# phuang1024/Starst3r

Hardware: AMD Instinct MI355X
Metric: 3DGS train iters/sec @ 1M Gaussians, 8x1080p views (higher is better)
Workload: dtype f32

## Files before the change

starst3r_amd/csrc/api.hip:

```cpp
#include <stdarg.h>

#include "common.h"

static thread_local char g_err[512] = "";

void st3r_set_error(const char* fmt, ...) {
    va_list ap;
    va_start(ap, fmt);
    vsnprintf(g_err, sizeof(g_err), fmt, ap);
    va_end(ap);
}

ST3R_EXPORT int st3r_version(void) { return ST3R_VERSION; }
ST3R_EXPORT const char* st3r_last_error(void) { return g_err; }

ST3R_EXPORT int st3r_ctx_create(int device, st3r_ctx** out) {
    ARG_CHECK(out);
    int ndev = 0;
    HIP_TRY(hipGetDeviceCount(&ndev));
    ARG_CHECK(device >= 0 && device < ndev);
    HIP_TRY(hipSetDevice(device));
    st3r_ctx* c = new (std::nothrow) st3r_ctx();
    if (!c) { st3r_set_error("out of host memory"); return ST3R_ERR_NOMEM; }
    memset(c, 0, sizeof(*c));
    c->device = device;
    hipError_t e = hipHostMalloc((void**)&c->pinned, 64 * sizeof(int64_t), hipHostMallocDefault);
    if (e != hipSuccess) { delete c; st3r_set_error("hipHostMalloc: %s", hipGetErrorString(e)); return ST3R_ERR_HIP; }
    *out = c;
    return ST3R_OK;
}

ST3R_EXPORT int st3r_ctx_destroy(st3r_ctx* ctx) {
    if (!ctx) return ST3R_OK;
    (void)hipSetDevice(ctx->device);
    (void)st3r_comm_destroy(ctx);
    for (int i = 0; i < SLOT_COUNT; ++i)
        if (ctx->slot_ptr[i]) (void)hipFree(ctx->slot_ptr[i]);
    if (ctx->pinned) (void)hipHostFree(ctx->pinned);
    if (ctx->count_event) (void)hipEventDestroy(ctx->count_event);
    if (ctx->peer_event) (void)hipEventDestroy(ctx->peer_event);
    if (ctx->comm_stream) {
        for (int j = 0; j < ST3R_MAX_RANGES; ++j) {
            (void)hipEventDestroy(ctx->ev_range_bwd[j]); (void)hipEventDestroy(ctx->ev_range_red[j]);
        }
        (void)hipStreamDestroy(ctx->comm_stream);
    }
    if (ctx->prof_ev[0][0][0])
        for (int r = 0; r < PROF_RING; ++r)
            for (int st = 0; st < STG_COUNT; ++st)
                for (int k = 0; k < 2; ++k) (void)hipEventDestroy(ctx->prof_ev[r][st][k]);
    delete ctx;
    return ST3R_OK;
}

ST3R_EXPORT int64_t st3r_ctx_arena_bytes(st3r_ctx* ctx) {
    if (!ctx) return 0;
    int64_t t = 0;
    for (int i = 0; i < SLOT_COUNT; ++i) t += (int64_t)ctx->slot_bytes[i];
    return t;
}

int st3r_arena_get(st3r_ctx* ctx, int slot, size_t bytes, void** out) {
    int grown;
    return st3r_arena_get2(ctx, slot, bytes, out, &grown);
}

int st3r_arena_get2(st3r_ctx* ctx, int slot, size_t bytes, void** out, int* grown) {
    *grown = 0;
    if (bytes == 0) bytes = 16;
    if (ctx->slot_bytes[slot] < bytes) {
        size_t want = bytes + bytes / 4;
        want = (want + 255) & ~(size_t)255;
        if (ctx->slot_ptr[slot]) {
            HIP_TRY(hipDeviceSynchronize());
            HIP_TRY(hipFree(ctx->slot_ptr[slot]));
            ctx->slot_ptr[slot] = nullptr; ctx->slot_bytes[slot] = 0;
        }
        hipError_t e = hipMalloc(&ctx->slot_ptr[slot], want);
        if (e != hipSuccess) {
            st3r_set_error("arena slot %d: hipMalloc(%zu) failed: %s", slot, want, hipGetErrorString(e));
            return ST3R_ERR_NOMEM;
        }
        ctx->slot_bytes[slot] = want;
        *grown = 1;
    }
    *out = ctx->slot_ptr[slot];
    return ST3R_OK;
}

ST3R_EXPORT int st3r_ctx_peek(st3r_ctx* ctx, void* stream, int which, void* dst, int64_t bytes) {
    ARG_CHECK(ctx && dst && bytes >= 0 && which >= 0 && which <= 10);
    static const int slots[11] = {SLOT_VALS_B, SLOT_OFFSETS, SLOT_SPLATS, SLOT_CUM,
                                  SLOT_MCMC_CUM, SLOT_MCMC_DEAD, SLOT_MCMC_SAMPLED, SLOT_MCMC_COUNT,
                                  SLOT_RGB, SLOT_ALPHA, SLOT_COUNTS};
    ARG_CHECK((size_t)bytes <= ctx->slot_bytes[slots[which]]);
    HIP_TRY(hipMemcpyAsync(dst, ctx->slot_ptr[slots[which]], (size_t)bytes, hipMemcpyDeviceToDevice,
                           (hipStream_t)stream));
    return ST3R_OK;
}

static const char* k_stage_names[STG_COUNT] = {"project", "scan", "emit", "sort", "offsets", "blend_fwd", "loss",
                                               "blend_bwd", "project_bwd", "adam", "sort_depth"};

ST3R_EXPORT const char* st3r_stage_name(int stage) {
    return (stage >= 0 && stage < STG_COUNT) ? k_stage_names[stage] : "";
}

static void prof_harvest_slot(st3r_ctx* ctx, int slot) {
    for (int st = 0; st < STG_COUNT; ++st) {
        if (!ctx->prof_used[slot][st]) continue;
        float ms = 0.f;
        if (hipEventSynchronize(ctx->prof_ev[slot][st][1]) == hipSuccess &&
            hipEventElapsedTime(&ms, ctx->prof_ev[slot][st][0], ctx->prof_ev[slot][st][1]) == hipSuccess) {
            ctx->prof_ms[st] += ms; ctx->prof_n[st] += 1;
        }
        ctx->prof_used[slot][st] = 0;
    }
}

void st3r_prof_begin(st3r_ctx* ctx, hipStream_t s, int stage) {
    if (!((ctx->prof_enabled >> stage) & 1)) return;
    (void)hipEventRecord(ctx->prof_ev[ctx->prof_slot][stage][0], s);
}

void st3r_prof_end(st3r_ctx* ctx, hipStream_t s, int stage) {
    if (!((ctx->prof_enabled >> stage) & 1)) return;
    (void)hipEventRecord(ctx->prof_ev[ctx->prof_slot][stage][1], s);
    ctx->prof_used[ctx->prof_slot][stage] = 1;
}

void st3r_prof_next_step(st3r_ctx* ctx) {
    if (!ctx->prof_enabled) return;
    ctx->prof_slot = (ctx->prof_slot + 1) % PROF_RING;
    prof_harvest_slot(ctx, ctx->prof_slot);
}

ST3R_EXPORT int st3r_ctx_set_debug(st3r_ctx* ctx, int flags) {
    ARG_CHECK(ctx);
    ctx->debug_flags = flags;
    return ST3R_OK;
}

ST3R_EXPORT int st3r_ctx_set_profiling(st3r_ctx* ctx, int enable) {
    ARG_CHECK(ctx && enable >= 0 && enable < 2 + STG_COUNT);
    if (enable && !ctx->prof_ev[0][0][0]) {
        for (int r = 0; r < PROF_RING; ++r)
            for (int st = 0; st < STG_COUNT; ++st)
                for (int k = 0; k < 2; ++k) HIP_TRY(hipEventCreate(&ctx->prof_ev[r][st][k]));
    }
    ctx->prof_enabled = enable == 0 ? 0 : (enable == 1 ? (1 << STG_COUNT) - 1 : (1 << (enable - 2)));
    return ST3R_OK;
}

ST3R_EXPORT int st3r_ctx_get_stage_ms(st3r_ctx* ctx, double* ms_out, int64_t* counts_out) {
    ARG_CHECK(ctx && ms_out && counts_out);
    HIP_TRY(hipDeviceSynchronize());
    if (ctx->prof_ev[0][0][0])
        for (int r = 0; r < PROF_RING; ++r) prof_harvest_slot(ctx, r);
    for (int st = 0; st < STG_COUNT; ++st) {
        ms_out[st] = ctx->prof_ms[st]; counts_out[st] = ctx->prof_n[st];
        ctx->prof_ms[st] = 0; ctx->prof_n[st] = 0;
    }
    return ST3R_OK;
}

int st3r_isect_scan_impl(st3r_ctx* ctx, hipStream_t s, int64_t n_pairs, const int32_t* tiles, int32_t* cum,
                         int64_t* n_isects_host, const void* pack_rects, int rect32, uint64_t* pack_out,
                         int32_t** total_dev_out, int32_t* total_copy, int32_t* total_host);
int st3r_isect_emit_impl(hipStream_t s, int N, int C, const float* splats, const int32_t* cum, int tile_size,
                         int tile_w, int tile_h, int64_t* isect_ids, int32_t* flatten_ids);
int st3r_sort_impl(st3r_ctx* ctx, hipStream_t s, int64_t n, int end_bit, int64_t* keys_in, int32_t* vals_in,
                   int64_t* keys_out, int32_t* vals_out);
int st3r_isect_offsets_impl(hipStream_t s, int64_t n_isects, const int64_t* ids, int C, int tile_w, int tile_h,
                            int32_t* offsets);
int st3r_project_impl(st3r_ctx* ctx, hipStream_t s, int N, int C, const float* means, const float* quats, const float* scales,
                      const float* opacities, const float* sh, int sh_stride, const float* viewmats, const float* Ks,
                      const float* campos, int width, int height, int tile_size, float eps2d, float near_plane,
                      float far_plane, float radius_clip, float* splats, int32_t* tiles_per_gauss, double* reg_sums,
                      uint64_t* depth_keys, int32_t* depth_vals, int tight, uint32_t key_base, void* rects, int rect32,
                      int reg_overwrite, double* zero_ptr, int zero_n, uint32_t* krange);
int st3r_sort_depth_seg_impl(st3r_ctx* ctx, hipStream_t s, int64_t N, int C, uint32_t* keys_in, int32_t* vals_in,
                             uint32_t* keys_out, int32_t* vals_out, const uint32_t* krange);
int st3r_isect_emit_chain_impl(st3r_ctx* ctx, hipStream_t s, int N, int C, const int32_t* perm, const void* rects,
                               int rect32, int tile_w, int tile_h, uint32_t* tile_keys, int32_t* vals, int64_t cap);
int st3r_records_prepare_impl(hipStream_t s, int N, int C, const float* splats, int tile_size, int tile_w, int tile_h,
                              int tight, int32_t* tiles, uint64_t* depth_keys, int32_t* depth_vals, uint32_t key_base,
                              void* rects, int rect32);
int st3r_isect_offsets32_impl(hipStream_t s, int64_t n_isects, const uint32_t* keys, int C, int tile_w, int tile_h,
                              int32_t* offsets, const int32_t* n_dev);
int st3r_sort_depth_impl(st3r_ctx* ctx, hipStream_t s, int64_t n, int end_bit, uint64_t* keys_in, int32_t* vals_in,
                         uint64_t* keys_out, int32_t* vals_out);
int st3r_sort_depth32_impl(st3r_ctx* ctx, hipStream_t s, int64_t n, int end_bit, uint32_t* keys_in, int32_t* vals_in,
                           uint32_t* keys_out, int32_t* vals_out);
int st3r_sort_tile_impl(st3r_ctx* ctx, hipStream_t s, int64_t n, int end_bit, uint32_t* keys_in, int32_t* vals_in,
                        uint32_t* keys_out, int32_t* vals_out, const int32_t* n_dev);
int st3r_blend_fwd_impl(st3r_ctx* ctx, hipStream_t s, int C, int W, int H, int tile_w, int tile_h,
                        const float* splats, const int32_t* offsets, const int32_t* flat, int64_t n_isects,
                        float* rgb, float* alpha, int32_t* last_ids, bool for_backward, bool end_in_offsets);
int st3r_blend_bwd_impl(st3r_ctx* ctx, hipStream_t s, int C, int W, int H, int tile_w, int tile_h,
                        const float* splats, const int32_t* offsets, const int32_t* flat, int64_t n_isects,
                        const float* alpha, const int32_t* last_ids, const float* v_rgb, const float* v_alpha,
                        const int32_t* cum, const uint64_t* rects, const uint64_t* rectbase, int tight, int64_t n_pairs,
                        float* v_splats,
                        bool end_in_offsets, st3r_vtile_ref* defer);
int st3r_project_sh_bwd_impl(hipStream_t s, int N, int C, const float* means, const float* quats, const float* scales,
                             const float* opacities, const float* sh, int sh_stride, const float* viewmats,
                             const float* Ks, const float* campos, int width, int height, float eps2d,
                             const float* splats, const float* v_splats, float reg_views, float opac_fac,
                             float scale_fac, float* grads, bool accumulate, int g_begin, int g_end, bool range_major,
                             const st3r_vtile_ref* slots);
int st3r_loss_impl(st3r_ctx* ctx, hipStream_t s, int C, int H, int W, const float* render, const float* gt,
                   float w_l1, float w_ssim, double* sums, float* v_render, bool sums_cleared);

static int bit_length_u32(uint32_t v) { int n = 0; while (v) { ++n; v >>= 1; } return n; }

static int settle_pending_count(st3r_ctx* ctx) {
    if (!ctx->count_pending) return ST3R_OK;
    HIP_TRY(hipEventSynchronize(ctx->count_event));
    ctx->count_pending = 0;
    const int64_t n = (int64_t)((int32_t*)(ctx->pinned + 8))[0];
    if (n < 0) {
        ctx->isect_hint = 0;
        ctx->view_chunks = (ctx->view_chunks > 0 ? ctx->view_chunks : 1) * 2;
        st3r_set_error("the previous step produced more than 2^31 tile intersections: its gradients were incomplete -- "
                       "repeat it (st3r_gs_train_fwd_bwd / st3r_gs_train_step now walk the views in %d chunks)",
                       ctx->view_chunks);
        return ST3R_ERR_CAPACITY;
    }
    if (n > ctx->count_cap) {
        ctx->isect_hint = 0;
        st3r_set_error("the previous step produced %lld tile intersections, more than the %lld its buffers were sized "
                       "for from the step before (+25 %%): its gradients were incomplete and st3r_adam_step / "
                       "st3r_gs_train_step did NOT apply them (the update is guarded on the device) -- repeat that step",
                       (long long)n, (long long)ctx->count_cap);
        return ST3R_ERR_CAPACITY;
    }
    ctx->isect_hint = n;
    return ST3R_OK;
}

int st3r_peer_status_settle(st3r_ctx* ctx);

ST3R_EXPORT int st3r_ctx_settle(st3r_ctx* ctx) {
    ARG_CHECK(ctx);
    int rc = st3r_peer_status_settle(ctx);
    if (rc) return rc;
    return settle_pending_count(ctx);
}

ST3R_EXPORT int st3r_ctx_release_scratch(st3r_ctx* ctx) {
    ARG_CHECK(ctx);
    HIP_TRY(hipDeviceSynchronize());
    const int rc = st3r_ctx_settle(ctx);
    for (int i = 0; i < SLOT_COUNT; ++i) {
        if (ctx->slot_ptr[i]) (void)hipFree(ctx->slot_ptr[i]);
        ctx->slot_ptr[i] = nullptr; ctx->slot_bytes[i] = 0;
    }
    return rc;
}

int st3r_counts_buffer(st3r_ctx* ctx, hipStream_t s, int32_t** out) {
    void* p; int grown = 0;
    int rc = st3r_arena_get2(ctx, SLOT_COUNTS, sizeof(int32_t) * 16, &p, &grown);
    if (rc) return rc;
    if (grown) HIP_TRY(hipMemsetAsync(p, 0, ctx->slot_bytes[SLOT_COUNTS], s));
    *out = (int32_t*)p;
    return ST3R_OK;
}

#define GET(slot, type, count, var)                                                          \
    type* var;                                                                               \
    {                                                                                        \
        void* _p;                                                                            \
        int _rc = st3r_arena_get(ctx, slot, sizeof(type) * (size_t)(count), &_p);            \
        if (_rc) return _rc;                                                                 \
        var = (type*)_p;                                                                     \
    }

struct RasterOut {
    float* splats; int32_t* offsets; int32_t* flat; int32_t* cum; const uint64_t* rects; uint64_t* rectbase;
    int64_t n_isects, n_records, n_isects_ref, n_visible; int tile_w, tile_h;
};

static int rasterize_front(st3r_ctx* ctx, hipStream_t s, int N, int C, const float* means, const float* quats,
                           const float* scales, const float* opacities, const float* sh, int sh_stride,
                           const float* viewmats, const float* Ks, const float* campos, int W, int H,
                           double* reg_sums, int tight, const float* records_in, bool allow_async, RasterOut* o,
                           double* loss_sums = nullptr) {
    const int tile = 16;
    const int tile_w = (W + tile - 1) / tile, tile_h = (H + tile - 1) / tile;
    const int64_t n_pairs = (int64_t)N * C;
    float* splats = const_cast<float*>(records_in);
    if (!records_in) {
        GET(SLOT_SPLATS, float, n_pairs * ST3R_SPLAT_STRIDE, own);
        splats = own;
    }
    GET(SLOT_CUM, int32_t, n_pairs, cum);
    GET(SLOT_OFFSETS, int32_t, (int64_t)C * tile_w * tile_h + 1, offsets);
    const float near_plane = 0.01f, far_plane = 1e10f;
    uint32_t near_bits, far_bits;
    memcpy(&near_bits, &near_plane, 4); memcpy(&far_bits, &far_plane, 4);
    const bool key32 = (C <= 8) && (far_bits - near_bits < 0x1FFFFFFFu);
    const int64_t n_sort = n_pairs;
    GET(SLOT_DKEYS_A, uint64_t, n_sort, dkeys_a);
    GET(SLOT_DKEYS_B, uint64_t, n_sort, dkeys_b);
    GET(SLOT_DVALS_A, int32_t, n_sort, dvals_a);
    GET(SLOT_DVALS_B, int32_t, n_sort, perm);
    const int rect32 = (tile_w <= 255 && tile_h <= 255 && !(ctx->debug_flags & 64)) ? 1 : 0;
    GET(SLOT_RECTS, uint64_t, rect32 ? (n_pairs + 1) / 2 : n_pairs, rects);
    int32_t* counts = nullptr;
    { int rc_ = st3r_counts_buffer(ctx, s, &counts); if (rc_) return rc_; }
    uint32_t* const krange = (key32 && reg_sums && !records_in && !(ctx->debug_flags & 4)) ? (uint32_t*)(counts + 8) : nullptr;
    st3r_prof_begin(ctx, s, STG_PROJECT);
    const uint32_t key_base = key32 ? near_bits : 0u;
    int rc = records_in
                 ? st3r_records_prepare_impl(s, N, C, splats, tile, tile_w, tile_h, tight, nullptr, dkeys_a, dvals_a,
                                             key_base, rects, rect32)
                 : st3r_project_impl(ctx, s, N, C, means, quats, scales, opacities, sh, sh_stride, viewmats, Ks, campos,
                                     W, H, tile, 0.3f, near_plane, far_plane, 0.0f, splats, nullptr, reg_sums, dkeys_a,
                                     dvals_a, tight, key_base, rects, rect32, 1, loss_sums, 2 * C, krange);
    if (!rc && records_in && loss_sums) HIP_TRY(hipMemsetAsync(loss_sums, 0, sizeof(double) * 2 * (size_t)C, s));
    st3r_prof_end(ctx, s, STG_PROJECT);
    if (rc) return rc;
    st3r_prof_begin(ctx, s, STG_SORT_DEPTH);
    const int cam_bits = bit_length_u32((uint32_t)(C - 1));
    rc = krange ? st3r_sort_depth_seg_impl(ctx, s, N, C, (uint32_t*)dkeys_a, dvals_a, (uint32_t*)dkeys_b, perm, krange)
         : key32 ? st3r_sort_depth32_impl(ctx, s, n_sort, 29 + cam_bits, (uint32_t*)dkeys_a, dvals_a, (uint32_t*)dkeys_b,
                                          perm)
                 : st3r_sort_depth_impl(ctx, s, n_sort, 32 + cam_bits, dkeys_a, dvals_a, dkeys_b, perm);
    st3r_prof_end(ctx, s, STG_SORT_DEPTH);
    if (rc) return rc;
    int64_t n_isects = 0;
    st3r_prof_begin(ctx, s, STG_SCAN);
    uint64_t* rectbase = nullptr;
    if (tile_w <= 1023 && tile_h <= 1023 && !(ctx->debug_flags & 64)) {
        GET(SLOT_RECTBASE, uint64_t, n_pairs, rb);
        rectbase = rb;
    }
    const int32_t* n_dev = nullptr;
    const int64_t sig = ((int64_t)N << 34) ^ ((int64_t)C << 26) ^ ((int64_t)W << 13) ^ (int64_t)H;
    const bool async = allow_async && ctx->isect_hint > 0 && ctx->hint_sig == sig;
    int32_t* total_dev = nullptr;
    rc = st3r_isect_scan_impl(ctx, s, n_pairs, nullptr, cum, nullptr, rects, rect32, rectbase, &total_dev,
                              async ? counts : nullptr, async ? (int32_t*)(ctx->pinned + 8) : nullptr);
    st3r_prof_end(ctx, s, STG_SCAN);
    if (rc) return rc;
    if (async) {
        if (!ctx->count_event) HIP_TRY(hipEventCreateWithFlags(&ctx->count_event, hipEventDisableTiming));
        HIP_TRY(hipEventRecord(ctx->count_event, s));
        n_isects = ctx->isect_hint + ctx->isect_hint / 4 + 1024;
        if (ctx->debug_flags & 8) n_isects = ctx->isect_hint / 2;
        if (n_isects > 2147483647LL) n_isects = 2147483647LL;
        ctx->count_pending = 1; ctx->count_cap = n_isects;
        o->n_visible = -1; o->n_isects_ref = -1;
    } else {
        HIP_TRY(hipMemcpyAsync(ctx->pinned, total_dev, sizeof(int32_t), hipMemcpyDeviceToHost, s));
        if (reg_sums) HIP_TRY(hipMemcpyAsync(ctx->pinned + 1, reg_sums + 2, 2 * sizeof(double), hipMemcpyDeviceToHost, s));
        HIP_TRY(hipStreamSynchronize(s));
        n_isects = (int64_t)((int32_t*)ctx->pinned)[0];
        if (n_isects < 0) {
            st3r_set_error("more than 2^31 tile intersections in one call: split the views over more calls / GPUs");
            return ST3R_SPLIT_VIEWS;
        }
        o->n_visible = reg_sums ? (int64_t)((double*)ctx->pinned)[1] : -1;
        o->n_isects_ref = reg_sums ? (int64_t)((double*)ctx->pinned)[2] : n_isects;
        if (allow_async) { ctx->isect_hint = n_isects; ctx->hint_sig = sig; }
    }
    GET(SLOT_KEYS_A, uint32_t, n_isects, tkeys_a);
    GET(SLOT_KEYS_B, uint32_t, n_isects, tkeys_b);
    GET(SLOT_VALS_A, int32_t, n_isects, vals_a);
    GET(SLOT_VALS_B, int32_t, n_isects, vals_b);
    n_dev = total_dev;
    o->n_records = async ? -1 : n_isects;
    if (n_isects > 0) {
        st3r_prof_begin(ctx, s, STG_EMIT);
        rc = st3r_isect_emit_chain_impl(ctx, s, N, C, perm, rects, rect32, tile_w, tile_h, tkeys_a, vals_a, n_isects);
        st3r_prof_end(ctx, s, STG_EMIT);
        if (rc) return rc;
        const int end_bit = bit_length_u32((uint32_t)((int64_t)C * tile_w * tile_h - 1));
        st3r_prof_begin(ctx, s, STG_SORT);
        rc = st3r_sort_tile_impl(ctx, s, n_isects, end_bit, tkeys_a, vals_a, tkeys_b, vals_b, n_dev);
        st3r_prof_end(ctx, s, STG_SORT);
        if (rc) return rc;
    }
    st3r_prof_begin(ctx, s, STG_OFFSETS);
    rc = st3r_isect_offsets32_impl(s, n_isects, tkeys_b, C, tile_w, tile_h, offsets, n_dev);
    st3r_prof_end(ctx, s, STG_OFFSETS);
    if (rc) return rc;
    o->splats = splats; o->offsets = offsets; o->flat = vals_b; o->cum = cum; o->rects = rect32 ? nullptr : rects;
    o->rectbase = rectbase;
    o->n_isects = n_isects;
    o->tile_w = tile_w; o->tile_h = tile_h;
    return ST3R_OK;
}

__global__ void k_finalize_loss(int C, const double* __restrict__ sums, const double* __restrict__ reg_sums,
                                double inv_px, double inv_cnt, double w_l1, double w_ssim, double reg_views,
                                double opac_k, double scale_k, float* __restrict__ loss_out) {
    if (threadIdx.x == 0 && blockIdx.x == 0) {
        double loss = 0;
        for (int c = 0; c < C; ++c) loss += w_l1 * sums[2 * c] * inv_px + w_ssim * (1.0 - sums[2 * c + 1] * inv_cnt);
        loss += reg_views * (opac_k * reg_sums[0] + scale_k * reg_sums[1]);
        loss_out[0] = (float)loss;
    }
}

static int train_views(st3r_ctx* ctx, hipStream_t s, int N, int C, const float* means, const float* quats,
                       const float* scales, const float* opacities, const float* sh, int sh_stride,
                       const float* viewmats, const float* Ks, const float* campos, const float* gt_images, int W, int H,
                       float ssim_fac, float opac_fac, float scale_fac, double* sums, double* reg_sums, bool allow_async,
                       bool accumulate, float* grads, RasterOut* ro_out) {
    const int64_t n_pairs = (int64_t)N * C, n_px = (int64_t)C * H * W;
    RasterOut ro;
    int rc = rasterize_front(ctx, s, N, C, means, quats, scales, opacities, sh, sh_stride, viewmats, Ks, campos, W, H,
                             reg_sums, 1, nullptr, allow_async, &ro, sums);
    if (rc) return rc;
    const bool eio = true;
    GET(SLOT_RGB, float, n_px * 3, rgb);
    GET(SLOT_ALPHA, float, n_px, alpha);
    GET(SLOT_LAST, int32_t, n_px, last);
    GET(SLOT_VRENDER, float, n_px * 3, v_rgb);
    float* const v_splats = nullptr;
    st3r_vtile_ref slots_{}; st3r_vtile_ref* const slots = &slots_;
    st3r_prof_begin(ctx, s, STG_BLEND_FWD);
    rc = st3r_blend_fwd_impl(ctx, s, C, W, H, ro.tile_w, ro.tile_h, ro.splats, ro.offsets, ro.flat, ro.n_isects, rgb,
                             alpha, last, true, eio);
    st3r_prof_end(ctx, s, STG_BLEND_FWD);
    if (rc) return rc;
    st3r_prof_begin(ctx, s, STG_LOSS);
    rc = st3r_loss_impl(ctx, s, C, H, W, rgb, gt_images, 1.0f - ssim_fac, ssim_fac, sums, v_rgb, true);
    st3r_prof_end(ctx, s, STG_LOSS);
    if (rc) return rc;
    st3r_prof_begin(ctx, s, STG_BLEND_BWD);
    rc = st3r_blend_bwd_impl(ctx, s, C, W, H, ro.tile_w, ro.tile_h, ro.splats, ro.offsets, ro.flat, ro.n_isects, alpha,
                             last, v_rgb, nullptr, ro.cum, (ctx->debug_flags & 2) ? nullptr : ro.rects,
                             (ctx->debug_flags & 2) ? nullptr : ro.rectbase, 1, n_pairs, v_splats,
                             eio, slots);
    st3r_prof_end(ctx, s, STG_BLEND_BWD);
    if (rc) return rc;
    st3r_prof_begin(ctx, s, STG_PROJECT_BWD);
    ctx->ranges_recorded = 0;
    if (ctx->n_ranges > 1 && ctx->comm_stream) {
        GET(SLOT_GSTAGE, float, (int64_t)23 * N, gstage);
        const int K = ctx->n_ranges;
        for (int j = 0; j < K && !rc; ++j) {
            const int g0 = (int)((int64_t)N * j / K), g1 = (int)((int64_t)N * (j + 1) / K);
            rc = st3r_project_sh_bwd_impl(s, N, C, means, quats, scales, opacities, sh, sh_stride, viewmats, Ks, campos, W,
                                          H, 0.3f, ro.splats, v_splats, (float)C, opac_fac, scale_fac, gstage, accumulate, g0,
                                          g1, true, slots);
            if (!rc) HIP_TRY(hipEventRecord(ctx->ev_range_bwd[j], s));
        }
        if (!rc) ctx->ranges_recorded = K;
    } else {
        rc = st3r_project_sh_bwd_impl(s, N, C, means, quats, scales, opacities, sh, sh_stride, viewmats, Ks, campos, W, H,
                                      0.3f, ro.splats, v_splats, (float)C, opac_fac, scale_fac, grads, accumulate, 0, -1,
                                      false, slots);
    }
    st3r_prof_end(ctx, s, STG_PROJECT_BWD);
    *ro_out = ro;
    return rc;
}

ST3R_EXPORT int st3r_gs_train_fwd_bwd(st3r_ctx* ctx, void* stream, int N, int C, const float* means,
                                      const float* quats, const float* scales, const float* opacities,
                                      const float* sh, int sh_stride, const float* viewmats, const float* Ks,
                                      const float* campos, const float* gt_images, int width, int height,
                                      float ssim_fac, float opac_fac, float scale_fac, float* grads,
                                      float* loss_out, int64_t* stats_host) {
    ARG_CHECK(ctx && N > 0 && C > 0 && C <= ST3R_MAX_VIEWS && width > 0 && height > 0 && sh_stride >= 12);
    ARG_CHECK((int64_t)N * C < 2147483647LL);
    ARG_CHECK(means && quats && scales && opacities && sh && viewmats && Ks && campos && gt_images && grads && loss_out);
    hipStream_t s = (hipStream_t)stream;
    const int W = width, H = height;
    GET(SLOT_SMALL, double, 2 * (size_t)C + 12, small);
    double* sums = small;
    double* reg_sums = small + 2 * C;
    double* reg_scratch = reg_sums + 4;
    st3r_prof_next_step(ctx);
    int rc = settle_pending_count(ctx);
    if (rc) return rc;
    int chunks = ctx->view_chunks > 0 ? ctx->view_chunks : 1;
    if ((ctx->debug_flags & 32) && chunks < 2) chunks = 2;
    if (chunks > C) chunks = C;
    int64_t st_vis = 0, st_is = 0, st_ref = 0;
    for (;;) {
        st_vis = st_is = st_ref = 0;
        bool first = true;
        for (int k = 0; k < chunks && !rc; ++k) {
            const int c0 = (int)((int64_t)k * C / chunks), c1 = (int)((int64_t)(k + 1) * C / chunks);
            if (c1 == c0) continue;
            double* rs = first ? reg_sums : reg_scratch;
            RasterOut ro;
            rc = train_views(ctx, s, N, c1 - c0, means, quats, scales, opacities, sh, sh_stride, viewmats + 16 * c0,
                             Ks + 9 * c0, campos + 3 * c0, gt_images + (int64_t)c0 * H * W * 3, W, H, ssim_fac, opac_fac,
                             scale_fac, sums + 2 * c0, rs, stats_host == nullptr && chunks == 1 && !ctx->comm, !first, grads,
                             &ro);
            if (!rc) { st_vis += ro.n_visible; st_is += ro.n_records; st_ref += ro.n_isects_ref; }
            first = false;
        }
        if (rc == ST3R_SPLIT_VIEWS && chunks < C) {
            chunks = chunks * 2 < C ? chunks * 2 : C;
            rc = ST3R_OK;
            continue;
        }
        break;
    }
    if (rc == ST3R_SPLIT_VIEWS) rc = ST3R_ERR_INVALID;
    if (rc) return rc;
    if (chunks > 1) ctx->view_chunks = chunks;
    const int Hi = H - 10, Wi = W - 10;
    const double cnt = (Hi > 0 && Wi > 0) ? (double)Hi * Wi * 3 : 0.0;
    hipLaunchKernelGGL(k_finalize_loss, dim3(1), dim3(64), 0, s, C, sums, reg_sums, 1.0 / ((double)H * W * 3),
                       cnt > 0 ? 1.0 / cnt : 0.0, (double)(1.0f - ssim_fac), (double)ssim_fac, (double)C,
                       (double)opac_fac / N, (double)scale_fac / (3.0 * N), loss_out);
    LAUNCH_CHECK();
    if (stats_host) {
        stats_host[0] = st_vis; stats_host[1] = st_is; stats_host[2] = st3r_ctx_arena_bytes(ctx);
        stats_host[3] = st_ref;
    }
    return ST3R_OK;
}

ST3R_EXPORT int st3r_gs_raster_train(st3r_ctx* ctx, void* stream, int N, int C, const float* records,
                                     const float* gt_images, int width, int height, float ssim_fac,
                                     float* v_records, float* loss_out, int64_t* stats_host) {
    ARG_CHECK(ctx && N > 0 && C > 0 && width > 0 && height > 0 && records && gt_images && v_records && loss_out);
    ARG_CHECK(C <= ST3R_MAX_VIEWS && (int64_t)N * C < 2147483647LL);
    hipStream_t s = (hipStream_t)stream;
    const int W = width, H = height;
    const int64_t n_pairs = (int64_t)N * C, n_px = (int64_t)C * H * W;
    GET(SLOT_SMALL, double, 2 * (size_t)C + 8, small);
    double* sums = small;
    double* reg_sums = small + 2 * C;
    HIP_TRY(hipMemsetAsync(reg_sums, 0, sizeof(double) * 4, s));
    st3r_prof_next_step(ctx);
    RasterOut ro;
    int rc = settle_pending_count(ctx);
    if (rc) return rc;
    rc = rasterize_front(ctx, s, N, C, nullptr, nullptr, nullptr, nullptr, nullptr, 0, nullptr, nullptr, nullptr, W, H,
                         nullptr, 1, records, stats_host == nullptr, &ro);
    if (rc == ST3R_SPLIT_VIEWS) rc = ST3R_ERR_INVALID;
    if (rc) return rc;
    GET(SLOT_RGB, float, n_px * 3, rgb);
    GET(SLOT_ALPHA, float, n_px, alpha);
    GET(SLOT_LAST, int32_t, n_px, last);
    GET(SLOT_VRENDER, float, n_px * 3, v_rgb);
    st3r_prof_begin(ctx, s, STG_BLEND_FWD);
    rc = st3r_blend_fwd_impl(ctx, s, C, W, H, ro.tile_w, ro.tile_h, ro.splats, ro.offsets, ro.flat, ro.n_isects, rgb,
                             alpha, last, true, true);
    st3r_prof_end(ctx, s, STG_BLEND_FWD);
    if (rc) return rc;
    st3r_prof_begin(ctx, s, STG_LOSS);
    rc = st3r_loss_impl(ctx, s, C, H, W, rgb, gt_images, 1.0f - ssim_fac, ssim_fac, sums, v_rgb, false);
    st3r_prof_end(ctx, s, STG_LOSS);
    if (rc) return rc;
    st3r_prof_begin(ctx, s, STG_BLEND_BWD);
    rc = st3r_blend_bwd_impl(ctx, s, C, W, H, ro.tile_w, ro.tile_h, ro.splats, ro.offsets, ro.flat, ro.n_isects, alpha,
                             last, v_rgb, nullptr, ro.cum, ro.rects, ro.rectbase, 1, n_pairs, v_records, true, nullptr);
    st3r_prof_end(ctx, s, STG_BLEND_BWD);
    if (rc) return rc;
    const int Hi = H - 10, Wi = W - 10;
    const double cnt = (Hi > 0 && Wi > 0) ? (double)Hi * Wi * 3 : 0.0;
    hipLaunchKernelGGL(k_finalize_loss, dim3(1), dim3(64), 0, s, C, sums, reg_sums, 1.0 / ((double)H * W * 3),
                       cnt > 0 ? 1.0 / cnt : 0.0, (double)(1.0f - ssim_fac), (double)ssim_fac, 0.0, 0.0, 0.0, loss_out);
    LAUNCH_CHECK();
    if (stats_host) {
        stats_host[0] = -1; stats_host[1] = ro.n_records; stats_host[2] = st3r_ctx_arena_bytes(ctx); stats_host[3] = -1;
    }
    return ST3R_OK;
}

ST3R_EXPORT int st3r_gs_render(st3r_ctx* ctx, void* stream, int N, int C, const float* means, const float* quats,
                               const float* scales, const float* opacities, const float* sh, int sh_stride,
                               const float* viewmats, const float* Ks, const float* campos, int width, int height,
                               float* rgb, float* alpha, int64_t* stats_host) {
    ARG_CHECK(ctx && N > 0 && C > 0 && width > 0 && height > 0 && sh_stride >= 12);
    ARG_CHECK(C <= ST3R_MAX_VIEWS && (int64_t)N * C < 2147483647LL);
    ARG_CHECK(means && quats && scales && opacities && sh && viewmats && Ks && campos && rgb && alpha);
    hipStream_t s = (hipStream_t)stream;
    RasterOut ro;
    int rc = settle_pending_count(ctx);
    if (rc) return rc;
    rc = rasterize_front(ctx, s, N, C, means, quats, scales, opacities, sh, sh_stride, viewmats, Ks, campos, width, height,
                         nullptr, 0, nullptr, false, &ro);
    if (rc == ST3R_SPLIT_VIEWS) rc = ST3R_ERR_INVALID;
    if (rc) return rc;
    GET(SLOT_LAST, int32_t, (int64_t)C * height * width, last);
    rc = st3r_blend_fwd_impl(ctx, s, C, width, height, ro.tile_w, ro.tile_h, ro.splats, ro.offsets, ro.flat,
                             ro.n_isects, rgb, alpha, last, false, true);
    if (rc) return rc;
    if (stats_host) {
        stats_host[0] = -1; stats_host[1] = ro.n_records; stats_host[2] = st3r_ctx_arena_bytes(ctx); stats_host[3] = 0;
    }
    return ST3R_OK;
}
```

starst3r_amd/csrc/common.h:

```cpp
#pragma once
#include <hip/hip_runtime.h>
#include <stdint.h>
#include <stdio.h>
#include <string.h>

#include "../../include/st3r.h"

#define ST3R_EXPORT extern "C" __attribute__((visibility("default")))

void st3r_set_error(const char* fmt, ...);

#define HIP_TRY(expr)                                                                              \
    do {                                                                                           \
        hipError_t _e = (expr);                                                                    \
        if (_e != hipSuccess) {                                                                    \
            st3r_set_error("%s:%d: %s -> %s", __FILE__, __LINE__, #expr, hipGetErrorString(_e));   \
            return ST3R_ERR_HIP;                                                                   \
        }                                                                                          \
    } while (0)

#define ARG_CHECK(cond)                                                                    \
    do {                                                                                   \
        if (!(cond)) {                                                                     \
            st3r_set_error("%s:%d: invalid argument: %s", __FILE__, __LINE__, #cond);      \
            return ST3R_ERR_INVALID;                                                       \
        }                                                                                  \
    } while (0)

#define LAUNCH_CHECK() HIP_TRY(hipGetLastError())

enum ArenaSlot {
    SLOT_SPLATS = 0,
    SLOT_TILES,
    SLOT_CUM,
    SLOT_KEYS_A,
    SLOT_KEYS_B,
    SLOT_VALS_A,
    SLOT_VALS_B,
    SLOT_OFFSETS,
    SLOT_RGB,
    SLOT_ALPHA,
    SLOT_LAST,
    SLOT_VRENDER,
    SLOT_VSPLATS,
    SLOT_SSIM_A,
    SLOT_SORT_TMP,
    SLOT_SCAN_TMP,
    SLOT_SMALL,
    SLOT_CMASK,
    SLOT_TILE_NB,
    SLOT_VTILE,
    SLOT_DKEYS_A,
    SLOT_DKEYS_B,
    SLOT_DVALS_A,
    SLOT_DVALS_B,
    SLOT_CUM_D,
    SLOT_NN_PART,
    SLOT_MCMC_CUM,
    SLOT_MCMC_DEAD,
    SLOT_MCMC_RANK,
    SLOT_MCMC_COUNT,
    SLOT_MCMC_SAMPLED,
    SLOT_MCMC_BINOMS,
    SLOT_REG_PART,
    SLOT_RECTS,
    SLOT_RECTS_D,
    SLOT_RECTBASE,
    SLOT_COUNTS,
    SLOT_PSTAGE,
    SLOT_GSTAGE,
    SLOT_ALIGN_CTL,
    SLOT_PAIR_TOUCH,
    SLOT_KRANGE_PART,
    SLOT_SCAN_CHAIN,
    SLOT_POSE_PART,
    SLOT_VTILE_DEPTH,
    SLOT_DEPTH_PART,
    SLOT_COUNT
};

enum Stage {
    STG_PROJECT = 0,
    STG_SCAN,
    STG_EMIT,
    STG_SORT,
    STG_OFFSETS,
    STG_BLEND_FWD,
    STG_LOSS,
    STG_BLEND_BWD,
    STG_PROJECT_BWD,
    STG_ADAM,
    STG_SORT_DEPTH,
    STG_COUNT
};
#define PROF_RING 64
#define ST3R_MAX_RANGES 8

#define ST3R_SPLIT_VIEWS 1000

struct st3r_vtile_ref { const int32_t* cum; const float* vtile; int stamp; unsigned vt_cap; const uint32_t* touch; };

struct st3r_ctx {
    int device;
    void* slot_ptr[SLOT_COUNT];
    size_t slot_bytes[SLOT_COUNT];
    int64_t* pinned;
    int debug_flags;
    const float* gtm_gt; const float* gtm_mom; int gtm_c, gtm_h, gtm_w;
    int bwd_stamp;
    int depth_stamp;
    uint32_t scan_gen;
    int64_t isect_hint, count_cap;
    int64_t hint_sig;
    int count_pending;
    int view_chunks;
    hipEvent_t count_event;
    void* comm;
    int comm_owned, comm_rank, comm_size;
    int exchange;
    int comm_broken;
    int peer_pending;
    hipEvent_t peer_event;
    hipStream_t comm_stream;
    hipEvent_t ev_range_bwd[ST3R_MAX_RANGES], ev_range_red[ST3R_MAX_RANGES];
    void* xwin;
    int n_ranges;
    int ranges_recorded;
    int prof_enabled;
    hipEvent_t prof_ev[PROF_RING][STG_COUNT][2];
    unsigned char prof_used[PROF_RING][STG_COUNT];
    int prof_slot;
    double prof_ms[STG_COUNT];
    int64_t prof_n[STG_COUNT];
};

void st3r_prof_begin(st3r_ctx* ctx, hipStream_t s, int stage);
void st3r_prof_end(st3r_ctx* ctx, hipStream_t s, int stage);
void st3r_prof_next_step(st3r_ctx* ctx);

int st3r_arena_get(st3r_ctx* ctx, int slot, size_t bytes, void** out);
int st3r_arena_get2(st3r_ctx* ctx, int slot, size_t bytes, void** out, int* grown);

static inline int ceil_div(int64_t a, int64_t b) { return (int)((a + b - 1) / b); }
```

starst3r_amd/csrc/gs_blend.hip:

```cpp
#include <type_traits>

#include "common.h"
#include "tile_rect.h"
#include "blend_common.h"



struct TileGeom {
    int lb, cam, i, j, start, end, tx0, ty0;
    bool inside;
    float px, py;
};

__device__ __forceinline__ TileGeom tile_geom(int C, int W, int H, int tile_w, int tile_h,
                                              const int32_t* __restrict__ offsets, int n_isects) {
    TileGeom g;
    const int n_tiles = tile_w * tile_h, total = C * n_tiles;
        g.lb = xcd_remap(blockIdx.x, total, XCD_GROUP(C, n_tiles, tile_w));
    g.cam = g.lb / n_tiles;
    const int tile = g.lb - g.cam * n_tiles;
    const int ty = tile / tile_w, tx = tile - ty * tile_w;
    g.tx0 = tx * 16; g.ty0 = ty * 16;
    const int w = threadIdx.x >> 6, lane = threadIdx.x & 63;
    g.j = g.tx0 + ((w & 1) << 3) + (lane & 7);
    g.i = g.ty0 + ((w >> 1) << 3) + (lane >> 3);
    g.inside = (g.i < H) && (g.j < W);
    g.px = (float)g.j + 0.5f; g.py = (float)g.i + 0.5f;
    g.start = offsets[g.lb];
    g.end = (g.lb == total - 1 && n_isects >= 0) ? n_isects : offsets[g.lb + 1];
    return g;
}

__device__ __forceinline__ int stage_record(const float4* __restrict__ splats, int64_t id, int t, int tx0, int ty0,
                                            float4* sR) {
    const float4 a = splats[id * 3 + 0];
    const float4 b = splats[id * 3 + 1];
    const float4 c = splats[id * 3 + 2];
    stage_qform(a, b, c, t, sR);
    EllipseTest et;
    if (!ellipse_prepare(a.z, a.w, b.x, b.y, &et)) return 0;
    const float rx = ((float)tx0 + 0.5f) - a.x, ry = ((float)ty0 + 0.5f) - a.y;
    int rel = 0;
#pragma unroll
    for (int q = 0; q < 4; ++q) {
        const float dx0 = rx + (float)((q & 1) * 8), dy0 = ry + (float)((q >> 1) * 8);
        rel |= ellipse_hits_square(et, dx0, dx0 + 7.0f, dy0, dy0 + 7.0f) ? (1 << q) : 0;
    }
    return rel;
}

template <bool TRAIN>
__global__ __launch_bounds__(BLK) void k_blend_fwd(int C, int W, int H, int tile_w, int tile_h,
                                                   const float4* __restrict__ splats,
                                                   const int32_t* __restrict__ offsets,
                                                   const int32_t* __restrict__ flat, int n_isects,
                                                   float* __restrict__ out_rgb, float* __restrict__ out_alpha,
                                                   int32_t* __restrict__ last_ids,
                                                   uint64_t* __restrict__ cmask, int64_t cmask_words,
                                                   int32_t* __restrict__ tile_nb, int no_cull) {
    __shared__ float4 sR[BLK * 3];
    __shared__ uint64_t sMask[4][4];
    const TileGeom g = tile_geom(C, W, H, tile_w, tile_h, offsets, n_isects);
    const int w = threadIdx.x >> 6, lane = threadIdx.x & 63;
    float thr = g.inside ? 1.f / 255.f : __builtin_inff();
    float T = 1.0f, r = 0.f, gg = 0.f, b = 0.f;
    int cur = TRAIN ? 0x7fffffff : 0;
    int nb = 0;
    const int64_t mbase = mask_base(g.lb, g.start);
    for (int bs = g.start; bs < g.end; bs += BLK, ++nb) {
        if (__syncthreads_and(thr > 1.0f)) break;
        const int idx = bs + threadIdx.x;
        int rel = 0;
        if (idx < g.end) {
            rel = stage_record(splats, flat[idx], threadIdx.x, g.tx0, g.ty0, sR);
            if (no_cull) rel = 0xF;
        }
        const uint64_t m0 = __ballot(rel & 1), m1 = __ballot(rel & 2), m2 = __ballot(rel & 4), m3 = __ballot(rel & 8);
        if (lane == 0) { sMask[0][w] = m0; sMask[1][w] = m1; sMask[2][w] = m2; sMask[3][w] = m3; }
        __syncthreads();
#pragma unroll 1
        for (int jj = 0; jj < 4; ++jj) {
            uint64_t m64 = uniform_u64(sMask[w][jj]);
            uint64_t contributed = 0;
            if (__builtin_amdgcn_ballot_w64(thr < 1.0f) == 0) m64 = 0;
#pragma unroll 1
            for (int hh = 0; hh < 2; ++hh) {
            uint32_t m = hh ? (uint32_t)(m64 >> 32) : (uint32_t)m64;
            uint32_t cont32 = 0;
            while (m) {
                const int bit = __builtin_ctz(m);
                m &= m - 1;
                const int t = jj * 64 + hh * 32 + bit;
                const float4 a = sR[3 * t];
                const float4 q = sR[3 * t + 1];
                const float cb = sR[3 * t + 2].x;
                const float dx = a.x - g.px, dy = a.y - g.py;
                const float P = blend_power(dx, dy, a.w, q.x, q.y);
                const float al0 = fminf(0.999f, a.z * __builtin_amdgcn_exp2f(P));
                uint64_t okm = 0;
                bool ok = false;
                float al;
                if (TRAIN) {
                    okm = mask_not_positive(P) & mask_not_less(al0, thr);
                    al = zero_unless(okm, al0);
                } else {
                    ok = !(P > 0.f) && !(al0 < thr);
                    al = ok ? al0 : 0.f;
                }
                const float nT = T * (1.0f - al);
                const bool stop = nT <= 1e-4f;
                float vis = al * T;
                uint64_t tm;
                if (TRAIN) {
                    tm = okm;
                    float Tn = nT;
                    if (__builtin_expect(__builtin_amdgcn_ballot_w64(stop) != 0, 0)) {
                        thr = stop ? __builtin_inff() : thr;
                        vis = stop ? 0.0f : vis;
                        Tn = stop ? T : nT;
                        cur = stop ? bs + t : cur;
                        tm = okm & ~__builtin_amdgcn_ballot_w64(stop);
                    }
                    T = Tn;
                } else {
                    thr = stop ? __builtin_inff() : thr;
                    al = stop ? 0.0f : al;
                    vis = al * T;
                    T = stop ? T : nT;
                    const bool took = al > 0.0f;
                    cur = took ? bs + t : cur;
                    tm = __builtin_amdgcn_ballot_w64(took);
                }
                r = __builtin_fmaf(q.z, vis, r); gg = __builtin_fmaf(q.w, vis, gg); b = __builtin_fmaf(cb, vis, b);
                cont32 |= tm ? (1u << bit) : 0u;
            }
            contributed |= (uint64_t)cont32 << (32 * hh);
            }
            if (cmask && lane == 0) cmask[(int64_t)w * cmask_words + mbase + nb * 4 + jj] = contributed;
        }
    }
    if (g.inside) {
        const int64_t p = ((int64_t)g.cam * H + g.i) * W + g.j;
        out_rgb[3 * p] = r; out_rgb[3 * p + 1] = gg; out_rgb[3 * p + 2] = b;
        out_alpha[p] = 1.0f - T;
        last_ids[p] = TRAIN ? (cur == 0x7fffffff ? cur : cur - 1) : cur;
    }
    if (tile_nb && threadIdx.x == 0) tile_nb[g.lb] = nb;
}

static int hand_off_buffers(st3r_ctx* ctx, int C, int tile_w, int tile_h, int64_t n_isects, uint64_t** cmask,
                            int64_t* words, int32_t** tile_nb) {
    const int64_t total = (int64_t)C * tile_w * tile_h;
    *words = (n_isects >> 6) + 4 * total + 8;
    void* p;
    int rc = st3r_arena_get(ctx, SLOT_CMASK, sizeof(uint64_t) * 4 * (size_t)*words, &p);
    if (rc) return rc;
    *cmask = (uint64_t*)p;
    rc = st3r_arena_get(ctx, SLOT_TILE_NB, sizeof(int32_t) * (size_t)total, &p);
    if (rc) return rc;
    *tile_nb = (int32_t*)p;
    return ST3R_OK;
}

int st3r_blend_fwd_cells_impl(st3r_ctx* ctx, hipStream_t s, int C, int W, int H, int tile_w, int tile_h,
                              const float* splats, const int32_t* offsets, const int32_t* flat, float* rgb, float* alpha,
                              int32_t* last_ids, uint64_t* cmask, int64_t cmask_words, int32_t* tile_nb);

int st3r_blend_fwd_impl(st3r_ctx* ctx, hipStream_t s, int C, int W, int H, int tile_w, int tile_h,
                        const float* splats, const int32_t* offsets, const int32_t* flat, int64_t n_isects,
                        float* rgb, float* alpha, int32_t* last_ids, bool for_backward, bool end_in_offsets) {
    const int total = C * tile_w * tile_h;
    uint64_t* cmask = nullptr; int64_t words = 0; int32_t* tile_nb = nullptr;
    if (for_backward) {
        int rc = hand_off_buffers(ctx, C, tile_w, tile_h, n_isects, &cmask, &words, &tile_nb);
        if (rc) return rc;
    }
    if ((for_backward && end_in_offsets && !(ctx->debug_flags & 128)) || (end_in_offsets && (ctx->debug_flags & 512)))
        return st3r_blend_fwd_cells_impl(ctx, s, C, W, H, tile_w, tile_h, splats, offsets, flat, rgb, alpha, last_ids, cmask,
                                         words, tile_nb);
    if (for_backward && end_in_offsets)
        hipLaunchKernelGGL(k_blend_fwd<true>, dim3(total), dim3(BLK), 0, s, C, W, H, tile_w, tile_h, (const float4*)splats,
                           offsets, flat, -1, rgb, alpha, last_ids, cmask, words, tile_nb, ctx->debug_flags & 1);
    else
        hipLaunchKernelGGL(k_blend_fwd<false>, dim3(total), dim3(BLK), 0, s, C, W, H, tile_w, tile_h, (const float4*)splats,
                           offsets, flat, end_in_offsets ? -1 : (int)n_isects, rgb, alpha, last_ids, cmask, words, tile_nb,
                           ctx->debug_flags & 1);
    LAUNCH_CHECK();
    return ST3R_OK;
}

ST3R_EXPORT int st3r_gs_blend_fwd(st3r_ctx* ctx, void* stream, int C, int width, int height, int tile_size,
                                  int tile_w, int tile_h, const float* splats, const int32_t* offsets,
                                  const int32_t* flatten_ids, int64_t n_isects, float* rgb, float* alpha,
                                  int32_t* last_ids) {
    ARG_CHECK(ctx && C > 0 && width > 0 && height > 0 && tile_size == 16);
    ARG_CHECK(tile_w == (width + 15) / 16 && tile_h == (height + 15) / 16);
    ARG_CHECK(splats && offsets && rgb && alpha && last_ids && n_isects >= 0 && n_isects < 2147483647LL);
    ARG_CHECK(n_isects == 0 || flatten_ids);
    return st3r_blend_fwd_impl(ctx, (hipStream_t)stream, C, width, height, tile_w, tile_h, splats, offsets,
                               flatten_ids, n_isects, rgb, alpha, last_ids, true, false);
}

__device__ __forceinline__ void bwd_phase2(const float2* __restrict__ pr, unsigned tpack, int cnt, int lane, const float4* sA, float* accw, float qxf_lane, float qyf_lane,
                                           const float (&pvr)[CHUNK], const float (&pvg)[CHUNK],
                                           const float (&pvb)[CHUNK]) {
    static_assert(CHUNK == 4, "one DPP row per record of the chunk");
    const int r = lane >> 4, part = lane & 15;
    wave_lds_sync();
    const int t = (tpack >> (8 * r)) & 0xFF;
    const float2 mean = *reinterpret_cast<const float2*>(&sA[t]);
    const float dy = mean.y - qyf_lane;
    const float2* src = pr + r * PAIR_STRIDE + PAIR_AT(part * CHUNK);
    float W0 = 0.f, W1 = 0.f, W2 = 0.f, Sr = 0.f, Sg = 0.f, Sb = 0.f;
#pragma unroll
    for (int i = 0; i < CHUNK; ++i) {
        const float2 v = src[i];
        W0 += v.x;
        if (i == 1) { W1 = v.x; W2 = v.x; }
        if (i > 1) { W1 = fmaf((float)i, v.x, W1); W2 = fmaf((float)(i * i), v.x, W2); }
        Sr = fmaf(v.y, pvr[i], Sr); Sg = fmaf(v.y, pvg[i], Sg); Sb = fmaf(v.y, pvb[i], Sb);
    }
    const float d0 = mean.x - qxf_lane;
    const float So = W0, Sx = fmaf(d0, W0, -W1), Sxx = fmaf(d0, Sx - W1, W2);
    const float Sy = So * dy, Sxy = Sx * dy, Syy = Sy * dy;
    float k0, k1, k2;
    reduce9_rows(Sx, Sy, So, Sxx, Sxy, Syy, Sr, Sg, Sb, k0, k1, k2);
    if (r < cnt && (lane & 3) == 0) {
        const int b = (lane >> 2) & 3;
        const int slot0 = ((b & 1) << 1) | (b >> 1);
        float* acc = accw + t * ACC_VALS;
        acc[slot0] = k0;
        acc[4 + slot0] = k1;
        if (b == 0) acc[8] = k2;
    }
    wave_lds_sync();
}

template <bool HAS_VA, bool TOUCH = false>
__global__ __launch_bounds__(BLK) __attribute__((amdgpu_waves_per_eu(8))) void k_blend_bwd(int C, int W, int H, int tile_w, int tile_h,
                                                   const float4* __restrict__ splats,
                                                   const int32_t* __restrict__ offsets,
                                                   const int32_t* __restrict__ flat, int n_isects,
                                                   const float* __restrict__ out_alpha,
                                                   const int32_t* __restrict__ last_ids,
                                                   const float* __restrict__ v_rgb,
                                                   const float* __restrict__ v_alpha,
                                                   const uint64_t* __restrict__ cmask, int64_t cmask_words,
                                                   const int32_t* __restrict__ tile_nb,
                                                   const int32_t* __restrict__ cum,
                                                   const uint64_t* __restrict__ rects,
                                                   const uint64_t* __restrict__ rectbase, int tight,
                                                   float* __restrict__ vtile, int stamp, unsigned vt_cap) {

    __shared__ float4 sA[HB];
    __shared__ float4 sB[HB];
    __shared__ float sC[HB];
    __shared__ float sAccW[4][HB * ACC_VALS];
    __shared__ float2 sPair[4][CHUNK * PAIR_STRIDE];
    __shared__ uint64_t sClampW;
    const TileGeom g = tile_geom(C, W, H, tile_w, tile_h, offsets, n_isects);
    const int nb = tile_nb[g.lb];
    if (nb == 0) return;
    const int w = threadIdx.x >> 6, lane = threadIdx.x & 63;
    const int64_t p = ((int64_t)g.cam * H + g.i) * W + g.j;
    float T_final = 1.0f, vr = 0.f, vg = 0.f, vb = 0.f, va = 0.f;
    int bin_final = -1;
    if (g.inside) {
        T_final = 1.0f - out_alpha[p];
        vr = v_rgb[3 * p]; vg = v_rgb[3 * p + 1]; vb = v_rgb[3 * p + 2];
        if (HAS_VA) va = v_alpha[p];
        bin_final = last_ids[p];
    }
    const bool chk_index = __builtin_amdgcn_ballot_w64(bin_final != 0x7fffffff) != 0;
    float2* pr = sPair[w];
    float* accw = sAccW[w];
    float pvr[CHUNK], pvg[CHUNK], pvb[CHUNK];
    const int pbase = (lane & 15) * CHUNK;
    {
        float* px = reinterpret_cast<float*>(pr);
        px[lane] = vr; px[64 + lane] = vg; px[128 + lane] = vb;
        wave_lds_sync();
#pragma unroll
        for (int i = 0; i < CHUNK; ++i) { pvr[i] = px[pbase + i]; pvg[i] = px[64 + pbase + i]; pvb[i] = px[128 + pbase + i]; }
        wave_lds_sync();
    }
    const float qxf = (float)(g.tx0 + ((w & 1) << 3) + (pbase & 7)) + 0.5f;
    const float qyf_part = (float)(g.ty0 + ((w >> 1) << 3) + (pbase >> 3)) + 0.5f;
    float k_big = 0x1p64f, k_neg_thr = -__int_as_float(0x3b808080) * 0x1p64f;
    asm volatile("" : "+v"(k_big), "+v"(k_neg_thr));
    float T = T_final;
    float bv = 0.f;
    const int64_t mbase = mask_base(g.lb, g.start);
    const uint64_t* wmask = cmask + (int64_t)__builtin_amdgcn_readfirstlane(w) * cmask_words + mbase;
    uint64_t m_next = wmask[(BLK / HB) * nb - 1];
    for (int hb = (BLK / HB) * nb - 1; hb >= 0; --hb) {
        const int bs = g.start + hb * HB;
        const int bsz = min(HB, g.end - bs);
        const uint64_t m_cur = m_next;
        if (hb > 0) m_next = wmask[hb - 1];
        if (bsz <= 0) continue;
        int my_u = -1, my_cb = 0;
        float my_op = 0.f, my_ca = 0.f, my_cbb = 0.f, my_cc = 0.f;
        if ((int)threadIdx.x < bsz) {
            const int t = threadIdx.x;
            const int64_t my_id = flat[bs + t];
            const int64_t word = mbase + hb;
#pragma unroll
            for (int ww = 0; ww < 4; ++ww) my_cb |= (int)((cmask[ww * cmask_words + word] >> (t & 63)) & 1ull) << ww;
            float4 a = make_float4(0.f, 0.f, 0.f, 0.f), b = a, c = a;
            if (my_cb)
            {
                a = splats[my_id * 3 + 0];
                b = splats[my_id * 3 + 1];
                c = splats[my_id * 3 + 2];
                sA[t] = make_float4(a.x, a.y, a.z, -0.5f * LOG2E * a.w);
                sB[t] = make_float4(-LOG2E * b.x, -0.5f * LOG2E * b.y, b.z, b.w);
                sC[t] = c.x;
            }
            const float det_ = a.w * b.y - b.x * b.x;
            const bool hard = my_cb && !(a.z <= 0.998f && a.w > 0.f && b.y > 0.f && det_ >= 2e-3f * (a.w * b.y));
            const uint64_t cw = __builtin_amdgcn_ballot_w64(hard);
            if (t == 0) sClampW = cw;
            if (my_cb && rectbase) {
                if (TOUCH) reinterpret_cast<uint32_t*>(const_cast<uint64_t*>(rects))[my_id] = (uint32_t)stamp;
                const uint64_t r = rectbase[my_id];
                const int x0 = (int)(r & 0x3FF), y0 = (int)((r >> 10) & 0x3FF), rw = (int)((r >> 20) & 0x3FF);
                my_u = (int)(r >> 32) + ((g.ty0 >> 4) - y0) * rw + ((g.tx0 >> 4) - x0);
                my_op = a.z; my_ca = a.w; my_cbb = b.x; my_cc = b.y;
            } else if (my_cb) {
                int x0, y0, rw;
                if (rects) {
                    const uint64_t r = rects[my_id];
                    x0 = (int)(r & 0xFFFF); y0 = (int)((r >> 16) & 0xFFFF); rw = (int)((r >> 32) & 0xFFFF);
                } else {
                    TileRect tr = ref_tile_rect(a.x, a.y, (float)__float_as_int(c.z), 16, tile_w, tile_h);
                    if (tight) tr = tight_tile_rect(tr, a.x, a.y, a.z, a.w, b.x, b.y);
                    x0 = tr.x0; y0 = tr.y0; rw = tr.x1 - tr.x0;
                }
                const int cum_excl = my_id == 0 ? 0 : cum[my_id - 1];
                my_u = cum_excl + ((g.ty0 >> 4) - y0) * rw + ((g.tx0 >> 4) - x0);
                my_op = a.z; my_ca = a.w; my_cbb = b.x; my_cc = b.y;
            }
        }
        __syncthreads();
        auto walk = [&](auto chk_tag, auto clamp_tag) {
            constexpr bool CHK = decltype(chk_tag)::value, CLAMP = decltype(clamp_tag)::value;
            uint64_t m = m_cur;
            while (m) {
                unsigned tpack = 0;
                int cnt = 0;
#pragma unroll
                for (int k = 0; k < CHUNK; ++k) {
                    if (m) {
                        const int t = 63 - __builtin_clzll(m);
                        m &= ~(1ull << t);
                        const float4 a = sA[t];
                        const float4 q = sB[t];
                        const float cb_ = sC[t];
                        const float dx = a.x - g.px, dy = a.y - g.py;
                        const float P = blend_power(dx, dy, a.w, q.x, q.y);
                        const float vis0 = __builtin_amdgcn_exp2f(P);
                        const float ov0 = a.z * vis0;
                        float alpha;
                        if (CLAMP) {
                            const float al0 = fminf(0.999f, ov0);
                            uint64_t okm = mask_not_positive(P) & mask_not_less(al0, 1.f / 255.f);
                            if (CHK) okm &= __builtin_amdgcn_ballot_w64(bs + t <= bin_final);
                            alpha = zero_unless(okm, al0);
                        } else {
                            float step;
                            asm("v_fma_f32 %0, %1, %2, %3 clamp" : "=v"(step) : "v"(ov0), "v"(k_big), "v"(k_neg_thr));
                            alpha = ov0 * step;
                            if (CHK) alpha = zero_unless(__builtin_amdgcn_ballot_w64(bs + t <= bin_final), alpha);
                        }
                        float alpha_u = alpha;
                        if (CLAMP) alpha_u = ov0 <= 0.999f ? alpha : 0.f;
                        const float ra = __builtin_amdgcn_rcpf(1.0f - alpha);
                        const float cv = q.z * vr + q.w * vg + cb_ * vb;
                        T *= ra;
                        const float fac = alpha * T;
                        float v_al = cv * T - bv * ra;
                        if (HAS_VA) v_al += T_final * ra * va;
                        bv += cv * fac;
                        pr[k * PAIR_STRIDE + PAIR_AT(lane)] = make_float2(alpha_u * v_al, fac);
                        tpack |= (unsigned)t << (8 * k);
                        cnt = k + 1;
                    }
                }
                bwd_phase2(pr, tpack, cnt, lane, sA, accw, qxf, qyf_part, pvr, pvg, pvb);
            }
        };
        const bool clamp_round = (uniform_u64(sClampW) & m_cur) != 0;
        if (chk_index) {
            if (clamp_round) walk(std::true_type{}, std::true_type{}); else walk(std::true_type{}, std::false_type{});
        } else {
            if (clamp_round) walk(std::false_type{}, std::true_type{}); else walk(std::false_type{}, std::false_type{});
        }
        __syncthreads();
        if (my_cb && (unsigned)my_u < vt_cap) {
            float acc[ACC_VALS];
#pragma unroll
            for (int k = 0; k < ACC_VALS; ++k) acc[k] = 0.f;
#pragma unroll
            for (int ww = 0; ww < 4; ++ww) {
                if (my_cb & (1 << ww)) {
#pragma unroll
                    for (int k = 0; k < ACC_VALS; ++k) acc[k] += sAccW[ww][threadIdx.x * ACC_VALS + k];
                }
            }
            const float sx = -acc[0], sy = -acc[1];
            float2* dst = reinterpret_cast<float2*>(vtile + (int64_t)my_u * VT_STRIDE);
            dst[0] = make_float2(my_ca * sx + my_cbb * sy, my_cbb * sx + my_cc * sy);
            dst[1] = make_float2(my_op != 0.f ? acc[2] / my_op : 0.f, -0.5f * acc[3]);
            dst[2] = make_float2(-acc[4], -0.5f * acc[5]);
            dst[3] = make_float2(acc[6], acc[7]);
            dst[4] = make_float2(acc[8], __int_as_float(stamp));
        }
    }
}

__global__ __launch_bounds__(256) void k_gather_vtile(int64_t n_pairs, const int32_t* __restrict__ cum,
                                                      const float* __restrict__ vtile, int stamp, unsigned vt_cap,
                                                      float4* __restrict__ v_splats) {
    constexpr int ROW = ACC_VALS;
    __shared__ int sCum[257];
    __shared__ float sVal[256 * ROW];
    const int tid = threadIdx.x;
    const int64_t p0 = (int64_t)blockIdx.x * 256;
    const int np = (int)min((int64_t)256, n_pairs - p0);
    if (tid == 0) sCum[0] = p0 == 0 ? 0 : cum[p0 - 1];
    sCum[tid + 1] = cum[p0 + min(tid, np - 1)];
    __syncthreads();
    const int s0 = sCum[0], s1 = sCum[np];
    const int my_start = sCum[tid], my_end = tid < np ? sCum[tid + 1] : sCum[tid];
    float acc[ACC_VALS];
#pragma unroll
    for (int k = 0; k < ACC_VALS; ++k) acc[k] = 0.f;
    float2 q0, q1, q2, q3, q4;
    auto fetch = [&](int u) {
        q0 = q1 = q2 = q3 = q4 = make_float2(0.f, 0.f);
        if (u < s1 && (unsigned)u < vt_cap) {
            const float2* src = reinterpret_cast<const float2*>(vtile + (int64_t)u * VT_STRIDE);
            q0 = src[0]; q1 = src[1]; q2 = src[2]; q3 = src[3]; q4 = src[4];
        }
    };
    fetch(s0 + tid);
    for (int base = s0; base < s1; base += 256) {
        const bool live = __float_as_int(q4.y) == stamp;
        float* row = sVal + tid * ROW;
        row[0] = live ? q0.x : 0.f; row[1] = live ? q0.y : 0.f; row[2] = live ? q1.x : 0.f;
        row[3] = live ? q1.y : 0.f; row[4] = live ? q2.x : 0.f; row[5] = live ? q2.y : 0.f;
        row[6] = live ? q3.x : 0.f; row[7] = live ? q3.y : 0.f; row[8] = live ? q4.x : 0.f;
        __syncthreads();
        fetch(base + 256 + tid);
        const int lo = max(my_start, base) - base, hi = min(my_end, base + 256) - base;
        for (int r = lo; r < hi; ++r) {
            const float* src = sVal + r * ROW;
#pragma unroll
            for (int k = 0; k < ACC_VALS; ++k) acc[k] += src[k];
        }
        __syncthreads();
    }
    if (tid < np) {
        const int64_t pid = p0 + tid;
        v_splats[pid * 3 + 0] = make_float4(acc[0], acc[1], acc[2], acc[3]);
        v_splats[pid * 3 + 1] = make_float4(acc[4], acc[5], acc[6], acc[7]);
        v_splats[pid * 3 + 2] = make_float4(acc[8], 0.f, 0.f, 0.f);
    }
}

int st3r_blend_bwd_impl(st3r_ctx* ctx, hipStream_t s, int C, int W, int H, int tile_w, int tile_h,
                        const float* splats, const int32_t* offsets, const int32_t* flat, int64_t n_isects,
                        const float* alpha, const int32_t* last_ids, const float* v_rgb, const float* v_alpha,
                        const int32_t* cum, const uint64_t* rects, const uint64_t* rectbase, int tight, int64_t n_pairs,
                        float* v_splats, bool end_in_offsets, st3r_vtile_ref* defer) {
    if (defer) *defer = st3r_vtile_ref{cum, nullptr, 0, 0u, nullptr};
    if (n_isects == 0) {
        if (!defer) HIP_TRY(hipMemsetAsync(v_splats, 0, sizeof(float) * ST3R_SPLAT_STRIDE * (size_t)n_pairs, s));
        return ST3R_OK;
    }
    uint64_t* cmask; int64_t words; int32_t* tile_nb;
    int rc = hand_off_buffers(ctx, C, tile_w, tile_h, n_isects, &cmask, &words, &tile_nb);
    if (rc) return rc;
    void* p; int grown = 0;
    rc = st3r_arena_get2(ctx, SLOT_VTILE, sizeof(float) * VT_STRIDE * (size_t)n_isects, &p, &grown);
    if (rc) return rc;
    float* vtile = (float*)p;
    uint32_t* touch = nullptr;
    int grown_t = 0;
    if (defer && rectbase && !v_alpha && n_isects > 8 * n_pairs) {
        void* pt;
        rc = st3r_arena_get2(ctx, SLOT_PAIR_TOUCH, sizeof(uint32_t) * (size_t)n_pairs, &pt, &grown_t);
        if (rc) return rc;
        touch = (uint32_t*)pt;
    }
    if (grown || ctx->bwd_stamp >= 2147483000) {
        HIP_TRY(hipMemsetAsync(p, 0, ctx->slot_bytes[SLOT_VTILE], s));
        if (ctx->slot_ptr[SLOT_PAIR_TOUCH])
            HIP_TRY(hipMemsetAsync(ctx->slot_ptr[SLOT_PAIR_TOUCH], 0, ctx->slot_bytes[SLOT_PAIR_TOUCH], s));
        ctx->bwd_stamp = 0;
    } else if (grown_t) {
        HIP_TRY(hipMemsetAsync(touch, 0, ctx->slot_bytes[SLOT_PAIR_TOUCH], s));
    }
    const int stamp = ++ctx->bwd_stamp;
    const int total = C * tile_w * tile_h;
    const unsigned vt_cap = (unsigned)(ctx->slot_bytes[SLOT_VTILE] / (sizeof(float) * VT_STRIDE));
    if (v_alpha)
        hipLaunchKernelGGL(k_blend_bwd<true>, dim3(total), dim3(BLK), 0, s, C, W, H, tile_w, tile_h,
                           (const float4*)splats, offsets, flat, end_in_offsets ? -1 : (int)n_isects, alpha, last_ids, v_rgb,
                           v_alpha, cmask, words, tile_nb, cum, rects, rectbase, tight, vtile, stamp, vt_cap);
    else if (touch)
        hipLaunchKernelGGL((k_blend_bwd<false, true>), dim3(total), dim3(BLK), 0, s, C, W, H, tile_w, tile_h,
                           (const float4*)splats, offsets, flat, end_in_offsets ? -1 : (int)n_isects, alpha, last_ids, v_rgb,
                           v_alpha, cmask, words, tile_nb, cum, reinterpret_cast<const uint64_t*>(touch), rectbase, tight, vtile,
                           stamp, vt_cap);
    else
        hipLaunchKernelGGL(k_blend_bwd<false>, dim3(total), dim3(BLK), 0, s, C, W, H, tile_w, tile_h,
                           (const float4*)splats, offsets, flat, end_in_offsets ? -1 : (int)n_isects, alpha, last_ids, v_rgb,
                           v_alpha, cmask, words, tile_nb, cum, rects, rectbase, tight, vtile, stamp, vt_cap);
    LAUNCH_CHECK();
    if (defer) { *defer = st3r_vtile_ref{cum, vtile, stamp, vt_cap, touch}; return ST3R_OK; }
    hipLaunchKernelGGL(k_gather_vtile, dim3(ceil_div(n_pairs, 256)), dim3(256), 0, s, n_pairs, cum, vtile, stamp, vt_cap,
                       (float4*)v_splats);
    LAUNCH_CHECK();
    return ST3R_OK;
}

ST3R_EXPORT int st3r_gs_blend_bwd(st3r_ctx* ctx, void* stream, int C, int width, int height, int tile_size,
                                  int tile_w, int tile_h, const float* splats, const int32_t* offsets,
                                  const int32_t* flatten_ids, int64_t n_isects, const float* alpha,
                                  const int32_t* last_ids, const float* v_rgb, const float* v_alpha,
                                  const int32_t* cum_tiles, int64_t n_pairs, float* v_splats) {
    ARG_CHECK(ctx && C > 0 && width > 0 && height > 0 && tile_size == 16);
    ARG_CHECK(tile_w == (width + 15) / 16 && tile_h == (height + 15) / 16);
    ARG_CHECK(splats && offsets && alpha && last_ids && v_rgb && v_splats && cum_tiles && n_pairs >= 0);
    ARG_CHECK(n_isects >= 0 && n_isects < 2147483647LL && (n_isects == 0 || flatten_ids));
    return st3r_blend_bwd_impl(ctx, (hipStream_t)stream, C, width, height, tile_w, tile_h, splats, offsets,
                               flatten_ids, n_isects, alpha, last_ids, v_rgb, v_alpha, cum_tiles, nullptr, nullptr, 0, n_pairs,
                               v_splats, false, nullptr);
}
```

starst3r_amd/csrc/gs_isect.hip:

```cpp
#include "common.h"
#include "tile_rect.h"

#define SCAN_THREADS 256
#define SCAN_ITEMS 16
#define SCAN_TILE (SCAN_THREADS * SCAN_ITEMS)

__device__ __forceinline__ int wave_incl_scan(int v) {
    const int lane = threadIdx.x & 63;
#pragma unroll
    for (int off = 1; off < 64; off <<= 1) {
        int t = __shfl_up(v, off);
        if (lane >= off) v += t;
    }
    return v;
}

__device__ __forceinline__ int block_incl_scan(int v, int* total) {
    __shared__ int wsum[4];
    const int lane = threadIdx.x & 63, w = threadIdx.x >> 6;
    int inc = wave_incl_scan(v);
    if (lane == 63) wsum[w] = inc;
    __syncthreads();
    int base = 0;
#pragma unroll
    for (int i = 0; i < 4; ++i) base += (i < w) ? wsum[i] : 0;
    *total = wsum[0] + wsum[1] + wsum[2] + wsum[3];
    __syncthreads();
    return inc + base;
}

typedef unsigned long long u64;
#define SCAN_PAD(i) ((i) + ((i) >> 5))
#define SC_VALUE_MASK 0xFFFFFFFFFFFFull
__device__ __forceinline__ u64 sc_word(u64 flag, uint32_t gen, u64 v) { return (flag << 62) | ((u64)gen << 48) | (v & SC_VALUE_MASK); }

__device__ __forceinline__ u64 chain_lookback256(const u64* st, int k, uint32_t gen, u64* s_part, int* s_near) {
    const int t = threadIdx.x, lane = t & 63, w = t >> 6;
    u64 excl = 0;
    for (int t0 = k - 1;; t0 -= 256) {
        const int tt = t0 - t;
        u64 wd = sc_word(2, gen, 0);
        if (tt >= 0) {
            unsigned spins = 0;
            for (;;) {
                wd = __hip_atomic_load(st + tt, __ATOMIC_RELAXED, __HIP_MEMORY_SCOPE_AGENT);
                if ((wd >> 62) != 0 && (uint32_t)((wd >> 48) & 0x3FFF) == gen) break;
                __builtin_amdgcn_s_sleep(1);
                if (++spins > (1u << 26)) __builtin_trap();
            }
        }
        const u64 incm = __ballot((wd >> 62) == 2);
        const int nearest = incm ? __builtin_ctzll(incm) : 64;
        u64 val = lane <= nearest ? (wd & SC_VALUE_MASK) : 0ull;
#pragma unroll
        for (int off = 32; off > 0; off >>= 1) val += __shfl_down(val, off);
        if (lane == 0) { s_part[w] = val; s_near[w] = nearest; }
        __syncthreads();
        bool done = false;
#pragma unroll
        for (int ww = 0; ww < 4; ++ww)
            if (!done) { excl += s_part[ww]; done = s_near[ww] < 64; }
        __syncthreads();
        if (done) break;
    }
    return excl;
}

template <bool RECTS, bool PACK>
__global__ __launch_bounds__(SCAN_THREADS) void k_scan_chained(const int32_t* in, const void* __restrict__ rects,
                                                               int rect32, int64_t n, int32_t* out,
                                                               uint64_t* __restrict__ pack_out, u64* status,
                                                               uint32_t* ticket, uint32_t gen,
                                                               int32_t* __restrict__ total_out,
                                                               int32_t* __restrict__ total_copy,
                                                               int32_t* __restrict__ total_host) {
    __shared__ int tile[SCAN_PAD(SCAN_TILE) + 1];
    __shared__ uint32_t s_tile;
    if (threadIdx.x == 0) {
        s_tile = atomicAdd(ticket + (gen & 1u), 1u);
        if (s_tile == 0) __hip_atomic_store(ticket + ((gen & 1u) ^ 1u), 0u, __ATOMIC_RELAXED, __HIP_MEMORY_SCOPE_AGENT);
    }
    __syncthreads();
    const uint32_t tl = s_tile;
    const int64_t base0 = (int64_t)tl * SCAN_TILE;
    if (base0 >= n) return;
    uint32_t geo[PACK ? SCAN_ITEMS : 1];
#pragma unroll
    for (int i = 0; i < SCAN_ITEMS; ++i) {
        const int e = i * SCAN_THREADS + threadIdx.x;
        const int64_t idx = base0 + e;
        int v = 0;
        if (RECTS) {
            uint32_t org = 0, rw = 0, rh = 0;
            if (idx < n) rect_load(rects, rect32, idx, &org, &rw, &rh);
            v = (int)(rw * rh);
            if (PACK) geo[i] = (org & 0x3FF) | (((org >> 16) & 0x3FF) << 10) | ((rw & 0x3FF) << 20);
        } else if (idx < n) v = in[idx];
        tile[SCAN_PAD(e)] = v;
    }
    __syncthreads();
    int v[SCAN_ITEMS];
    int s = 0;
#pragma unroll
    for (int i = 0; i < SCAN_ITEMS; ++i) {
        v[i] = tile[SCAN_PAD(threadIdx.x * SCAN_ITEMS + i)];
        s += v[i];
    }
    int total;
    const int inc = block_incl_scan(s, &total);
    const u64 tot = (u64)(uint32_t)total;
    __shared__ u64 s_part[4];
    __shared__ int s_near[4];
    u64 excl = 0;
    if (tl == 0) {
        if (threadIdx.x == 0) __hip_atomic_store(status, sc_word(2, gen, tot), __ATOMIC_RELAXED, __HIP_MEMORY_SCOPE_AGENT);
    } else {
        if (threadIdx.x == 0) __hip_atomic_store(status + tl, sc_word(1, gen, tot), __ATOMIC_RELAXED, __HIP_MEMORY_SCOPE_AGENT);
        excl = chain_lookback256(status, (int)tl, gen, s_part, s_near);
        if (threadIdx.x == 0)
            __hip_atomic_store(status + tl, sc_word(2, gen, excl + tot), __ATOMIC_RELAXED, __HIP_MEMORY_SCOPE_AGENT);
    }
    if (threadIdx.x == 0 && base0 + SCAN_TILE >= n) {
        const u64 all = excl + tot;
        total_out[0] = all > 2147483647ull ? -1 : (int32_t)all;
        if (total_copy) total_copy[0] = total_out[0];
        if (total_host) __hip_atomic_store(total_host, total_out[0], __ATOMIC_RELAXED, __HIP_MEMORY_SCOPE_SYSTEM);
    }
    const int tile_excl = (int)(uint32_t)excl;
    int run = tile_excl + inc - s;
#pragma unroll
    for (int i = 0; i < SCAN_ITEMS; ++i) {
        run += v[i];
        tile[SCAN_PAD(threadIdx.x * SCAN_ITEMS + i)] = run;
    }
    __syncthreads();
#pragma unroll
    for (int i = 0; i < SCAN_ITEMS; ++i) {
        const int e = i * SCAN_THREADS + threadIdx.x;
        const int64_t idx = base0 + e;
        if (idx < n) {
            out[idx] = tile[SCAN_PAD(e)];
            if (PACK) {
                const uint32_t ex = (uint32_t)(e == 0 ? tile_excl : tile[SCAN_PAD(e - 1)]);
                pack_out[idx] = ((uint64_t)ex << 32) | geo[i];
            }
        }
    }
}

struct ChainCtl { uint32_t* tickets; int32_t* total; u64* status; uint32_t gen; };
static int chain_ctl(st3r_ctx* ctx, hipStream_t s, int64_t nwords, ChainCtl* c) {
    void* p; int grown = 0;
    int rc = st3r_arena_get2(ctx, SLOT_SCAN_CHAIN, sizeof(u64) * ((size_t)nwords + 16), &p, &grown);
    if (rc) return rc;
    if (grown || ctx->scan_gen >= 0x3FFF) {
        HIP_TRY(hipMemsetAsync(p, 0, ctx->slot_bytes[SLOT_SCAN_CHAIN], s));
        ctx->scan_gen = 0;
    }
    u64* ctl = (u64*)p;
    c->gen = ++ctx->scan_gen;
    c->tickets = (uint32_t*)ctl;
    c->total = (int32_t*)(ctl + 4) + (c->gen & 3);
    c->status = ctl + 16;
    return ST3R_OK;
}

int st3r_scan_inclusive_i32(st3r_ctx* ctx, hipStream_t s, const int32_t* in, const void* rects, int rect32, int32_t* out,
                            int64_t n, int32_t** total_dev, uint64_t* pack_out = nullptr, int32_t* total_copy = nullptr,
                            int32_t* total_host = nullptr) {
    const int ntiles = ceil_div(n, SCAN_TILE);
    ChainCtl c;
    int rc = chain_ctl(ctx, s, ntiles, &c);
    if (rc) return rc;
#define SCAN_LAUNCH(R, P)                                                                                                \
    hipLaunchKernelGGL((k_scan_chained<R, P>), dim3(ntiles), dim3(SCAN_THREADS), 0, s, in, rects, rect32, n, out, pack_out, \
                       c.status, c.tickets, c.gen, c.total, total_copy, total_host)
    if (rects && pack_out) SCAN_LAUNCH(true, true);
    else if (rects) SCAN_LAUNCH(true, false);
    else SCAN_LAUNCH(false, false);
#undef SCAN_LAUNCH
    LAUNCH_CHECK();
    if (total_dev) *total_dev = c.total;
    return ST3R_OK;
}

int st3r_isect_scan_impl(st3r_ctx* ctx, hipStream_t s, int64_t n_pairs, const int32_t* tiles, int32_t* cum,
                         int64_t* n_isects_host, const void* pack_rects, int rect32, uint64_t* pack_out,
                         int32_t** total_dev_out, int32_t* total_copy, int32_t* total_host) {
    if (n_pairs == 0) { if (n_isects_host) *n_isects_host = 0; return ST3R_OK; }
    int32_t* total_dev = nullptr;
    int rc = st3r_scan_inclusive_i32(ctx, s, tiles, tiles ? nullptr : pack_rects, rect32, cum, n_pairs, &total_dev,
                                     tiles ? nullptr : pack_out, total_copy, total_host);
    if (rc) return rc;
    if (total_dev_out) *total_dev_out = total_dev;
    if (n_isects_host) {
        int32_t* pin = (int32_t*)ctx->pinned;
        HIP_TRY(hipMemcpyAsync(pin, total_dev, sizeof(int32_t), hipMemcpyDeviceToHost, s));
        HIP_TRY(hipStreamSynchronize(s));
        *n_isects_host = (int64_t)pin[0];
    }
    return ST3R_OK;
}

ST3R_EXPORT int st3r_gs_isect_scan(st3r_ctx* ctx, void* stream, int64_t n_pairs, const int32_t* tiles_per_gauss,
                                   int32_t* cum_tiles, int64_t* n_isects_host) {
    ARG_CHECK(ctx && n_pairs >= 0 && tiles_per_gauss && cum_tiles && n_isects_host);
    return st3r_isect_scan_impl(ctx, (hipStream_t)stream, n_pairs, tiles_per_gauss, cum_tiles, n_isects_host, nullptr,
                                0, nullptr, nullptr, nullptr, nullptr);
}

__global__ __launch_bounds__(256) void k_isect_emit(int N, int64_t n_pairs, const float4* __restrict__ splats,
                                                    const int32_t* __restrict__ cum, int tile_size, int tile_w,
                                                    int tile_h, int tile_n_bits, int64_t* __restrict__ isect_ids,
                                                    int32_t* __restrict__ flatten_ids) {
    const int64_t pid = (int64_t)blockIdx.x * blockDim.x + threadIdx.x;
    if (pid >= n_pairs) return;
    const int end = cum[pid];
    const int start = pid == 0 ? 0 : cum[pid - 1];
    if (end == start) return;
    const float4 r0 = splats[pid * 3 + 0];
    const float4 r2 = splats[pid * 3 + 2];
    const float radius = (float)__float_as_int(r2.z);
    const TileRect tr = ref_tile_rect(r0.x, r0.y, radius, tile_size, tile_w, tile_h);
    const int x0 = tr.x0, y0 = tr.y0, x1 = tr.x1, y1 = tr.y1;
    const int64_t cid = pid / N;
    const int64_t cid_enc = cid << (32 + tile_n_bits);
    const int64_t depth_enc = (int64_t)(uint32_t)__float_as_int(r2.y);
    int cur = start;
    for (int ty = y0; ty < y1; ++ty)
        for (int tx = x0; tx < x1; ++tx) {
            const int64_t tile_id = (int64_t)ty * tile_w + tx;
            isect_ids[cur] = cid_enc | (tile_id << 32) | depth_enc;
            flatten_ids[cur] = (int32_t)pid;
            ++cur;
        }
}

static int bit_length_u32(uint32_t v) { int n = 0; while (v) { ++n; v >>= 1; } return n; }

int st3r_isect_emit_impl(hipStream_t s, int N, int C, const float* splats, const int32_t* cum, int tile_size,
                         int tile_w, int tile_h, int64_t* isect_ids, int32_t* flatten_ids) {
    int64_t n_pairs = (int64_t)N * C;
    if (n_pairs == 0) return ST3R_OK;
    int tile_n_bits = bit_length_u32((uint32_t)(tile_w * tile_h));
    hipLaunchKernelGGL(k_isect_emit, dim3(ceil_div(n_pairs, 256)), dim3(256), 0, s, N, n_pairs, (const float4*)splats,
                       cum, tile_size, tile_w, tile_h, tile_n_bits, isect_ids, flatten_ids);
    LAUNCH_CHECK();
    return ST3R_OK;
}

ST3R_EXPORT int st3r_gs_isect_emit(st3r_ctx* ctx, void* stream, int N, int C, const float* splats,
                                   const int32_t* cum_tiles, int tile_size, int tile_w, int tile_h,
                                   int64_t n_isects, int64_t* isect_ids, int32_t* flatten_ids) {
    ARG_CHECK(ctx && N >= 0 && C > 0 && splats && cum_tiles && tile_size > 0 && tile_w > 0 && tile_h > 0);
    if (n_isects == 0) return ST3R_OK;
    ARG_CHECK(isect_ids && flatten_ids);
    return st3r_isect_emit_impl((hipStream_t)stream, N, C, splats, cum_tiles, tile_size, tile_w, tile_h, isect_ids,
                                flatten_ids);
}

__global__ __launch_bounds__(256) void k_isect_offsets(int64_t n_isects, const int64_t* __restrict__ ids, int C,
                                                       int n_tiles, int tile_n_bits,
                                                       int32_t* __restrict__ offsets) {
    const int64_t idx = (int64_t)blockIdx.x * blockDim.x + threadIdx.x;
    if (idx >= n_isects) return;
    const int64_t hi = ids[idx] >> 32;
    const int64_t id_curr = (hi >> tile_n_bits) * n_tiles + (hi & (((int64_t)1 << tile_n_bits) - 1));
    if (idx == 0) {
        for (int64_t i = 0; i <= id_curr; ++i) offsets[i] = 0;
    } else {
        const int64_t hp = ids[idx - 1] >> 32;
        const int64_t id_prev = (hp >> tile_n_bits) * n_tiles + (hp & (((int64_t)1 << tile_n_bits) - 1));
        if (id_prev != id_curr)
            for (int64_t i = id_prev + 1; i <= id_curr; ++i) offsets[i] = (int32_t)idx;
    }
    if (idx == n_isects - 1) {
        const int64_t total = (int64_t)C * n_tiles;
        for (int64_t i = id_curr + 1; i < total; ++i) offsets[i] = (int32_t)n_isects;
    }
}

int st3r_isect_offsets_impl(hipStream_t s, int64_t n_isects, const int64_t* ids, int C, int tile_w, int tile_h,
                            int32_t* offsets) {
    int n_tiles = tile_w * tile_h;
    if (n_isects == 0) {
        HIP_TRY(hipMemsetAsync(offsets, 0, sizeof(int32_t) * (size_t)C * n_tiles, s));
        return ST3R_OK;
    }
    int tile_n_bits = bit_length_u32((uint32_t)n_tiles);
    hipLaunchKernelGGL(k_isect_offsets, dim3(ceil_div(n_isects, 256)), dim3(256), 0, s, n_isects, ids, C, n_tiles,
                       tile_n_bits, offsets);
    LAUNCH_CHECK();
    return ST3R_OK;
}

ST3R_EXPORT int st3r_gs_offsets(st3r_ctx* ctx, void* stream, int64_t n_isects, const int64_t* isect_ids_sorted,
                                int C, int tile_w, int tile_h, int32_t* offsets) {
    ARG_CHECK(ctx && n_isects >= 0 && C > 0 && tile_w > 0 && tile_h > 0 && offsets);
    ARG_CHECK(n_isects == 0 || isect_ids_sorted);
    return st3r_isect_offsets_impl((hipStream_t)stream, n_isects, isect_ids_sorted, C, tile_w, tile_h, offsets);
}

__global__ __launch_bounds__(256) void k_isect_offsets32(int64_t n_isects, const uint32_t* __restrict__ keys,
                                                         int64_t total, int32_t* __restrict__ offsets,
                                                         const int32_t* __restrict__ n_dev) {
    if (n_dev) n_isects = min(n_isects, (int64_t)max(*n_dev, 0));
    const int64_t tid = (int64_t)blockIdx.x * blockDim.x + threadIdx.x;
    if (n_isects == 0) {
        for (int64_t i = tid; i <= total; i += (int64_t)gridDim.x * blockDim.x) offsets[i] = 0;
        return;
    }
    const int64_t i0 = tid * 4;
    if (i0 >= n_isects) return;
    uint32_t k[4];
    if (i0 + 4 <= n_isects) {
        const uint4 v = *reinterpret_cast<const uint4*>(keys + i0);
        k[0] = v.x; k[1] = v.y; k[2] = v.z; k[3] = v.w;
    } else {
#pragma unroll
        for (int j = 0; j < 4; ++j) k[j] = i0 + j < n_isects ? keys[i0 + j] : 0u;
    }
    int64_t prev = i0 == 0 ? -1 : (int64_t)keys[i0 - 1];
#pragma unroll
    for (int j = 0; j < 4; ++j) {
        const int64_t idx = i0 + j;
        if (idx < n_isects) {
            const int64_t cur = k[j];
            for (int64_t i = prev + 1; i <= cur; ++i) offsets[i] = (int32_t)idx;
            prev = cur;
            if (idx == n_isects - 1)
                for (int64_t i = cur + 1; i <= total; ++i) offsets[i] = (int32_t)n_isects;
        }
    }
}

int st3r_isect_offsets32_impl(hipStream_t s, int64_t n_isects, const uint32_t* keys, int C, int tile_w, int tile_h,
                              int32_t* offsets, const int32_t* n_dev) {
    const int64_t total = (int64_t)C * tile_w * tile_h;
    if (n_isects == 0 && !n_dev) {
        HIP_TRY(hipMemsetAsync(offsets, 0, sizeof(int32_t) * (size_t)(total + 1), s));
        return ST3R_OK;
    }
    hipLaunchKernelGGL(k_isect_offsets32, dim3(ceil_div(n_isects > 0 ? (n_isects + 3) / 4 : 1, 256)), dim3(256), 0, s, n_isects,
                       keys, total, offsets, n_dev);
    LAUNCH_CHECK();
    return ST3R_OK;
}

__global__ __launch_bounds__(256) void k_records_prepare(int N, int64_t n_pairs, const float4* __restrict__ splats,
                                                         int tile_size, int tile_w, int tile_h, int tight,
                                                         int32_t* __restrict__ tiles, uint64_t* __restrict__ depth_keys,
                                                         int32_t* __restrict__ depth_vals, uint32_t key_base,
                                                         void* __restrict__ rects, int rect32) {
    const int64_t pid = (int64_t)blockIdx.x * blockDim.x + threadIdx.x;
    if (pid >= n_pairs) return;
    const float4 r2 = splats[pid * 3 + 2];
    const int radius = __float_as_int(r2.z);
    int ntiles = 0;
    TileRect tr = {0, 0, 0, 0};
    if (radius > 0) {
        const float4 r0 = splats[pid * 3 + 0];
        tr = ref_tile_rect(r0.x, r0.y, (float)radius, tile_size, tile_w, tile_h);
        if (tight) {
            const float4 r1 = splats[pid * 3 + 1];
            tr = tight_tile_rect(tr, r0.x, r0.y, r0.z, r0.w, r1.x, r1.y);
        }
        ntiles = (tr.y1 - tr.y0) * (tr.x1 - tr.x0);
    }
    if (tiles) tiles[pid] = ntiles;
    if (rects) rect_store(rects, rect32, pid, tr);
    const uint32_t dbits = radius > 0 ? (uint32_t)__float_as_int(r2.y) : 0xFFFFFFFFu;
    if (key_base)
        reinterpret_cast<uint32_t*>(depth_keys)[pid] =
            ((uint32_t)(pid / N) << 29) | (radius > 0 ? dbits - key_base : 0x1FFFFFFFu);
    else
        depth_keys[pid] = ((uint64_t)(pid / N) << 32) | dbits;
    depth_vals[pid] = (int32_t)pid;
}

int st3r_records_prepare_impl(hipStream_t s, int N, int C, const float* splats, int tile_size, int tile_w, int tile_h,
                              int tight, int32_t* tiles, uint64_t* depth_keys, int32_t* depth_vals, uint32_t key_base,
                              void* rects, int rect32) {
    const int64_t n_pairs = (int64_t)N * C;
    if (n_pairs == 0) return ST3R_OK;
    hipLaunchKernelGGL(k_records_prepare, dim3(ceil_div(n_pairs, 256)), dim3(256), 0, s, N, n_pairs,
                       (const float4*)splats, tile_size, tile_w, tile_h, tight, tiles, depth_keys, depth_vals, key_base,
                       rects, rect32);
    LAUNCH_CHECK();
    return ST3R_OK;
}


#ifndef EP
#define EP 1024
#endif
#define EPT (EP / 256)
#define ECH 4096

__device__ __forceinline__ void emit_item(int C, int bpc, int* c, int* k) {
    const int b = blockIdx.x;
    if ((C & 7) == 0) { const int j = b >> 3; *c = (b & 7) + 8 * (j / bpc); *k = j % bpc; }
    else { *c = b / bpc; *k = b % bpc; }
}

__global__ __launch_bounds__(256) void k_isect_gather(int N, int C, int bpc, const int32_t* __restrict__ perm,
                                                      const void* __restrict__ rects, int rect32,
                                                      void* __restrict__ rects_d, int32_t* __restrict__ wg_tiles) {
    int c, k;
    emit_item(C, bpc, &c, &k);
    const int t = threadIdx.x;
    const int64_t first = (int64_t)c * N + (int64_t)k * EP;
    const int np = (int)min((int64_t)EP, (int64_t)(c + 1) * N - first);
    int32_t pid[EPT];
#pragma unroll
    for (int j = 0; j < EPT; ++j) pid[j] = j * 256 + t < np ? perm[first + j * 256 + t] : -1;
    int sum = 0;
#pragma unroll
    for (int j = 0; j < EPT; ++j) {
        if (pid[j] >= 0) {
            const int64_t dst = first + j * 256 + t;
            if (rect32) {
                const uint32_t r = reinterpret_cast<const uint32_t*>(rects)[pid[j]];
                reinterpret_cast<uint32_t*>(rects_d)[dst] = r;
                sum += (int)((r >> 16) & 0xFFu) * (int)(r >> 24);
            } else {
                const uint64_t r = reinterpret_cast<const uint64_t*>(rects)[pid[j]];
                reinterpret_cast<uint64_t*>(rects_d)[dst] = r;
                sum += (int)((r >> 32) & 0xFFFF) * (int)(r >> 48);
            }
        }
    }
    int total;
    block_incl_scan(sum, &total);
    if (t == 0) wg_tiles[c * bpc + k] = total;
}

#define EMIT_SELF_BASE_MAX 16384
__global__ __launch_bounds__(1024) void k_isect_wg_scan(int n, const int32_t* __restrict__ wg_tiles,
                                                        long long* __restrict__ wg_base) {
    __shared__ long long s_wave[16];
    const int t = threadIdx.x, lane = t & 63, w = t >> 6;
    const int per = (n + 1023) / 1024;
    const int e0 = min(t * per, n), e1 = min(e0 + per, n);
    long long sum = 0;
    for (int e = e0; e < e1; ++e) sum += wg_tiles[e];
    long long inc = sum;
#pragma unroll
    for (int off = 1; off < 64; off <<= 1) {
        const long long o = __shfl_up(inc, off);
        if (lane >= off) inc += o;
    }
    if (lane == 63) s_wave[w] = inc;
    __syncthreads();
    long long base = 0;
#pragma unroll
    for (int i = 0; i < 16; ++i) base += i < w ? s_wave[i] : 0;
    long long run = base + inc - sum;
    for (int e = e0; e < e1; ++e) { wg_base[e] = run; run += wg_tiles[e]; }
}

__global__ __launch_bounds__(256) void k_isect_emit_d(int N, int C, int bpc, const int32_t* __restrict__ perm,
                                                      const void* __restrict__ rects_d, int rect32,
                                                      const long long* __restrict__ wg_base,
                                                      const int32_t* __restrict__ wg_tiles, int tile_w, int tile_h,
                                                      uint32_t* __restrict__ tile_keys, int32_t* __restrict__ vals,
                                                      int64_t cap) {
    __shared__ int s_end[EP];
    __shared__ uint32_t s_org[EP];
    __shared__ uint16_t s_w[EP];
    __shared__ int32_t s_pid[EP];
    __shared__ uint16_t s_own[ECH];
    __shared__ unsigned s_wmax[4];
    __shared__ long long s_bsum[4];
    int c, k;
    emit_item(C, bpc, &c, &k);
    const int t = threadIdx.x, lane = t & 63, w = t >> 6;
    long long bsum = 0;
    if (!wg_base) {
        const int nb4 = (c * bpc + k) >> 2;
        for (int i = t; i < nb4; i += 256) {
            const int4 v = reinterpret_cast<const int4*>(wg_tiles)[i];
            bsum += ((long long)v.x + v.y) + ((long long)v.z + v.w);
        }
        if (t < ((c * bpc + k) & 3)) bsum += wg_tiles[4 * nb4 + t];
    }
    const int64_t first = (int64_t)c * N + (int64_t)k * EP;
    const int np = (int)min((int64_t)EP, (int64_t)(c + 1) * N - first);
    int cnt[EPT];
#pragma unroll
    for (int j = 0; j < EPT; ++j) {
        const int e = j * 256 + t;
        int32_t pid = 0;
        uint32_t org = 0, rw = 0, rh = 0;
        if (e < np) {
            pid = perm[first + e];
            rect_load(rects_d, rect32, first + e, &org, &rw, &rh);
        }
        s_pid[e] = pid; s_org[e] = org; s_w[e] = (uint16_t)rw;
        cnt[j] = (int)(rw * rh);
    }
    int carry = 0;
#pragma unroll
    for (int j = 0; j < EPT; ++j) {
        int tot;
        const int inc = block_incl_scan(cnt[j], &tot);
        s_end[j * 256 + t] = carry + inc;
        carry += tot;
    }
    const int total = carry;
    __syncthreads();
    long long base;
    if (wg_base) base = wg_base[c * bpc + k];
    else {
#pragma unroll
        for (int off = 32; off > 0; off >>= 1) bsum += __shfl_down(bsum, off);
        if (lane == 0) s_bsum[w] = bsum;
        __syncthreads();
        base = (s_bsum[0] + s_bsum[1]) + (s_bsum[2] + s_bsum[3]);
    }
    const uint32_t key0 = (uint32_t)c * (uint32_t)(tile_w * tile_h);
    int carry_owner = 0;
    for (int c0 = 0; c0 < total; c0 += ECH) {
        reinterpret_cast<uint4*>(s_own)[t] = make_uint4(0u, 0u, 0u, 0u);
        reinterpret_cast<uint4*>(s_own)[t + 256] = make_uint4(0u, 0u, 0u, 0u);
        __syncthreads();
#pragma unroll
        for (int j = 0; j < EPT; ++j) {
            const int e = j * 256 + t;
            if (e < np) {
                const int start = e ? s_end[e - 1] : 0;
                if (s_end[e] > start && start >= c0 && start < c0 + ECH) s_own[start - c0] = (uint16_t)(e + 1);
            }
        }
        __syncthreads();
        uint4 a = reinterpret_cast<const uint4*>(s_own)[2 * t], b = reinterpret_cast<const uint4*>(s_own)[2 * t + 1];
        unsigned wv[8] = {a.x, a.y, a.z, a.w, b.x, b.y, b.z, b.w};
        unsigned run = 0;
#pragma unroll
        for (int i = 0; i < 8; ++i) {
            const unsigned lo = max(run, wv[i] & 0xFFFFu);
            run = max(lo, wv[i] >> 16);
            wv[i] = lo | (run << 16);
        }
        unsigned inc = run;
#pragma unroll
        for (int off = 1; off < 64; off <<= 1) {
            const unsigned o = __shfl_up(inc, off);
            if (lane >= off) inc = max(inc, o);
        }
        if (lane == 63) s_wmax[w] = inc;
        unsigned excl_m = __shfl_up(inc, 1);
        if (lane == 0) excl_m = 0;
        __syncthreads();
        unsigned pre = max((unsigned)carry_owner, excl_m);
#pragma unroll
        for (int ww = 0; ww < 4; ++ww)
            if (ww < w) pre = max(pre, s_wmax[ww]);
        carry_owner = (int)max(max(max((unsigned)carry_owner, s_wmax[0]), max(s_wmax[1], s_wmax[2])), s_wmax[3]);
#pragma unroll
        for (int i = 0; i < 8; ++i) {
            const unsigned lo = max(wv[i] & 0xFFFFu, pre), hi = max(wv[i] >> 16, pre);
            wv[i] = lo | (hi << 16);
        }
        reinterpret_cast<uint4*>(s_own)[2 * t] = make_uint4(wv[0], wv[1], wv[2], wv[3]);
        reinterpret_cast<uint4*>(s_own)[2 * t + 1] = make_uint4(wv[4], wv[5], wv[6], wv[7]);
        __syncthreads();
        const int lim = min(ECH, total - c0);
        for (int i = t; i < lim; i += 256) {
            const int p = (int)s_own[i] - 1;
            const int o = c0 + i;
            const int kk = o - (p == 0 ? 0 : s_end[p - 1]);
            const uint32_t w_ = s_w[p], org = s_org[p];
            int qq = (int)((float)kk * __builtin_amdgcn_rcpf((float)w_));
            int rem = kk - qq * (int)w_;
            if (rem < 0) { --qq; rem += (int)w_; }
            if (rem >= (int)w_) { ++qq; rem -= (int)w_; }
            const uint32_t tx = (org & 0xFFFF) + (uint32_t)rem, ty = (org >> 16) + (uint32_t)qq;
            const long long pos = base + o;
            if (pos >= 0 && pos < cap) {
                tile_keys[pos] = key0 + ty * (uint32_t)tile_w + tx;
                vals[pos] = s_pid[p];
            }
        }
        __syncthreads();
    }
}

int st3r_isect_emit_chain_impl(st3r_ctx* ctx, hipStream_t s, int N, int C, const int32_t* perm, const void* rects,
                               int rect32, int tile_w, int tile_h, uint32_t* tile_keys, int32_t* vals, int64_t cap) {
    const int64_t n_pairs = (int64_t)N * C;
    if (n_pairs == 0) return ST3R_OK;
    const int bpc = ceil_div(N, EP);
    const int grid = C * bpc;
    void* p;
    int rc = st3r_arena_get(ctx, SLOT_RECTS_D, (rect32 ? sizeof(uint32_t) : sizeof(uint64_t)) * (size_t)n_pairs, &p);
    if (rc) return rc;
    void* rects_d = p;
    rc = st3r_arena_get(ctx, SLOT_CUM_D, (sizeof(long long) + sizeof(int32_t)) * (size_t)grid + 16, &p);
    if (rc) return rc;
    long long* wg_base = (long long*)p;
    int32_t* wg_tiles = (int32_t*)(wg_base + grid);
    if (((uintptr_t)wg_tiles & 15) != 0) wg_tiles += 2;
    hipLaunchKernelGGL(k_isect_gather, dim3(grid), dim3(256), 0, s, N, C, bpc, perm, rects, rect32, rects_d, wg_tiles);
    const bool self_base = grid <= EMIT_SELF_BASE_MAX;
    if (!self_base) hipLaunchKernelGGL(k_isect_wg_scan, dim3(1), dim3(1024), 0, s, grid, wg_tiles, wg_base);
    hipLaunchKernelGGL(k_isect_emit_d, dim3(grid), dim3(256), 0, s, N, C, bpc, perm, rects_d, rect32,
                       self_base ? (const long long*)nullptr : wg_base, wg_tiles, tile_w, tile_h, tile_keys, vals, cap);
    LAUNCH_CHECK();
    return ST3R_OK;
}
```

starst3r_amd/csrc/gs_project.hip:

```cpp
#include "common.h"
#include "tile_rect.h"

#define CAM_STRIDE 32

__device__ __forceinline__ float dot3f(float a0, float a1, float a2, float b0, float b1, float b2) {
    return (a0 * b0 + a1 * b1) + a2 * b2;
}

#define SH_C0 0.2820947917738781f
#define SH_C1 0.48860251190292f

__global__ __launch_bounds__(256) void k_project_sh_fwd(
    int N, int C, const float* __restrict__ means, const float* __restrict__ quats,
    const float* __restrict__ scales, const float* __restrict__ opacities, const float* __restrict__ sh,
    int sh_stride, const float* __restrict__ viewmats, const float* __restrict__ Ks,
    const float* __restrict__ campos, int W, int H, int tile_size, int tile_w, int tile_h, float eps2d,
    float near_plane, float far_plane, float radius_clip, float4* __restrict__ splats,
    int32_t* __restrict__ tiles_per_gauss, double* __restrict__ reg_part,
    uint64_t* __restrict__ depth_keys, int32_t* __restrict__ depth_vals, int tight, uint32_t key_base,
    void* __restrict__ rects, int rect32, uint32_t* __restrict__ krange_part) {
    extern __shared__ float cam[];
    __shared__ float red[8];
    for (int c = threadIdx.x; c < C; c += blockDim.x) {
        float* o = cam + c * CAM_STRIDE;
        const float* V = viewmats + 16 * c;
        for (int k = 0; k < 12; ++k) o[k] = V[k];
        const float* K = Ks + 9 * c;
        float fx = K[0], fy = K[4], cx = K[2], cy = K[5];
        o[12] = fx; o[13] = fy; o[14] = cx; o[15] = cy;
        float tan_fovx = 0.5f * (float)W / fx;
        float tan_fovy = 0.5f * (float)H / fy;
        o[16] = ((float)W - cx) / fx + 0.3f * tan_fovx;
        o[17] = cx / fx + 0.3f * tan_fovx;
        o[18] = ((float)H - cy) / fy + 0.3f * tan_fovy;
        o[19] = cy / fy + 0.3f * tan_fovy;
        o[20] = campos[3 * c]; o[21] = campos[3 * c + 1]; o[22] = campos[3 * c + 2];
    }
    __syncthreads();

    const int g = blockIdx.x * blockDim.x + threadIdx.x;
    const bool active = g < N;
    float mx = 0, my = 0, mz = 0, opac = 0;
    float cov0 = 0, cov1 = 0, cov2 = 0, cov3 = 0, cov4 = 0, cov5 = 0;
    float k[12];
    float reg_o = 0.f, reg_s = 0.f;
    if (active) {
        mx = means[3 * g]; my = means[3 * g + 1]; mz = means[3 * g + 2];
        opac = opacities[g];
        float qw = quats[4 * g], qx = quats[4 * g + 1], qy = quats[4 * g + 2], qz = quats[4 * g + 3];
        float s0 = scales[3 * g], s1 = scales[3 * g + 1], s2 = scales[3 * g + 2];
        const float* kp = sh + (int64_t)g * sh_stride;
#pragma unroll
        for (int i = 0; i < 12; ++i) k[i] = kp[i];
        float n2 = ((qw * qw + qx * qx) + qy * qy) + qz * qz;
        float inv = 1.0f / sqrtf(n2);
        qw *= inv; qx *= inv; qy *= inv; qz *= inv;
        float x2 = qx * qx, y2 = qy * qy, z2 = qz * qz;
        float xy = qx * qy, xz = qx * qz, yz = qy * qz;
        float wx = qw * qx, wy = qw * qy, wz = qw * qz;
        float m0 = (1.0f - 2.0f * (y2 + z2)) * s0, m1 = (2.0f * (xy - wz)) * s1, m2 = (2.0f * (xz + wy)) * s2;
        float m3 = (2.0f * (xy + wz)) * s0, m4 = (1.0f - 2.0f * (x2 + z2)) * s1, m5 = (2.0f * (yz - wx)) * s2;
        float m6 = (2.0f * (xz - wy)) * s0, m7 = (2.0f * (yz + wx)) * s1, m8 = (1.0f - 2.0f * (x2 + y2)) * s2;
        cov0 = dot3f(m0, m1, m2, m0, m1, m2);
        cov1 = dot3f(m0, m1, m2, m3, m4, m5);
        cov2 = dot3f(m0, m1, m2, m6, m7, m8);
        cov3 = dot3f(m3, m4, m5, m3, m4, m5);
        cov4 = dot3f(m3, m4, m5, m6, m7, m8);
        cov5 = dot3f(m6, m7, m8, m6, m7, m8);
        if (reg_part) {
            reg_o = 1.0f / (1.0f + __expf(-opac));
            reg_s = (__expf(s0) + __expf(s1)) + __expf(s2);
        }
    }
    if (reg_part) {
        for (int off = 32; off > 0; off >>= 1) {
            reg_o += __shfl_down(reg_o, off);
            reg_s += __shfl_down(reg_s, off);
        }
        int w = threadIdx.x >> 6;
        if ((threadIdx.x & 63) == 0) { red[w] = reg_o; red[4 + w] = reg_s; }
        __syncthreads();
        if (threadIdx.x == 0) {
            reg_part[4 * blockIdx.x + 0] = (double)((red[0] + red[1]) + (red[2] + red[3]));
            reg_part[4 * blockIdx.x + 1] = (double)((red[4] + red[5]) + (red[6] + red[7]));
        }
    }
    int n_vis = 0, n_ref = 0;
    uint32_t kmin = 0xFFFFFFFFu, kmax = 0u;
    for (int c = 0; active && c < C; ++c) {
        const float* o = cam + c * CAM_STRIDE;
        const float R00 = o[0], R01 = o[1], R02 = o[2], t0 = o[3];
        const float R10 = o[4], R11 = o[5], R12 = o[6], t1 = o[7];
        const float R20 = o[8], R21 = o[9], R22 = o[10], t2 = o[11];
        const int64_t pid = (int64_t)c * N + g;
        float x = dot3f(R00, R01, R02, mx, my, mz) + t0;
        float y = dot3f(R10, R11, R12, mx, my, mz) + t1;
        float z = dot3f(R20, R21, R22, mx, my, mz) + t2;
        bool valid = !(z < near_plane || z > far_plane);
        float m2x = 0, m2y = 0, ca = 0, cb = 0, cc = 0, radius = 0;
        if (valid) {
            float T0 = dot3f(R00, R01, R02, cov0, cov1, cov2), T1 = dot3f(R00, R01, R02, cov1, cov3, cov4),
                  T2 = dot3f(R00, R01, R02, cov2, cov4, cov5);
            float T3 = dot3f(R10, R11, R12, cov0, cov1, cov2), T4 = dot3f(R10, R11, R12, cov1, cov3, cov4),
                  T5 = dot3f(R10, R11, R12, cov2, cov4, cov5);
            float T6 = dot3f(R20, R21, R22, cov0, cov1, cov2), T7 = dot3f(R20, R21, R22, cov1, cov3, cov4),
                  T8 = dot3f(R20, R21, R22, cov2, cov4, cov5);
            float c0 = dot3f(T0, T1, T2, R00, R01, R02);
            float c1 = dot3f(T0, T1, T2, R10, R11, R12);
            float c2 = dot3f(T0, T1, T2, R20, R21, R22);
            float c3 = dot3f(T3, T4, T5, R10, R11, R12);
            float c4 = dot3f(T3, T4, T5, R20, R21, R22);
            float c5 = dot3f(T6, T7, T8, R20, R21, R22);
            const float fx = o[12], fy = o[13], cx = o[14], cy = o[15];
            float rz = 1.0f / z;
            float rz2 = rz * rz;
            float xr = x * rz, yr = y * rz;
            float tx = z * fminf(o[16], fmaxf(-o[17], xr));
            float ty = z * fminf(o[18], fmaxf(-o[19], yr));
            float a = fx * rz, cj = -(fx * tx) * rz2;
            float b = fy * rz, d = -(fy * ty) * rz2;
            float t0x = a * c0 + cj * c2;
            float t0y = a * c1 + cj * c4;
            float t0z = a * c2 + cj * c5;
            float t1y = b * c3 + d * c4;
            float t1z = b * c4 + d * c5;
            float c00 = t0x * a + t0z * cj;
            float c01 = t0y * b + t0z * d;
            float c11 = t1y * b + t1z * d;
            m2x = (fx * x) * rz + cx;
            m2y = (fy * y) * rz + cy;
            c00 += eps2d; c11 += eps2d;
            float det = c00 * c11 - c01 * c01;
            if (det <= 0.0f) valid = false;
            else {
                float inv_det = 1.0f / det;
                ca = c11 * inv_det; cb = -c01 * inv_det; cc = c00 * inv_det;
                float bb = 0.5f * (c00 + c11);
                float v1 = bb + sqrtf(fmaxf(0.01f, bb * bb - det));
                radius = ceilf(3.0f * sqrtf(v1));
                if (radius <= radius_clip) valid = false;
                else if (m2x + radius <= 0.0f || m2x - radius >= (float)W || m2y + radius <= 0.0f ||
                         m2y - radius >= (float)H)
                    valid = false;
            }
        }
        float4 r0 = make_float4(0, 0, 0, 0), r1 = r0, r2 = r0;
        int ntiles = 0;
        TileRect tr = {0, 0, 0, 0};
        if (valid) {
            float dx = mx - o[20], dy = my - o[21], dz = mz - o[22];
            float inorm = 1.0f / sqrtf((dx * dx + dy * dy) + dz * dz);
            dx *= inorm; dy *= inorm; dz *= inorm;
            float col[3];
#pragma unroll
            for (int ch = 0; ch < 3; ++ch) {
                float r = SH_C0 * k[ch];
                r = r + SH_C1 * ((-dy * k[3 + ch] + dz * k[6 + ch]) - dx * k[9 + ch]);
                r = r + 0.5f;
                col[ch] = r < 0.0f ? 0.0f : r;
            }
            tr = ref_tile_rect(m2x, m2y, radius, tile_size, tile_w, tile_h);
            n_ref += (tr.y1 - tr.y0) * (tr.x1 - tr.x0);
            if (tight) tr = tight_tile_rect(tr, m2x, m2y, opac, ca, cb, cc);
            ntiles = (tr.y1 - tr.y0) * (tr.x1 - tr.x0);
            r0 = make_float4(m2x, m2y, opac, ca);
            r1 = make_float4(cb, cc, col[0], col[1]);
            r2 = make_float4(col[2], z, __int_as_float((int)radius), 0.0f);
        }
        splats[pid * 3 + 0] = r0;
        splats[pid * 3 + 1] = r1;
        splats[pid * 3 + 2] = r2;
        if (tiles_per_gauss) tiles_per_gauss[pid] = ntiles;
        if (rects) rect_store(rects, rect32, pid, tr);
        if (depth_keys) {
            const uint32_t dbits = valid ? (uint32_t)__float_as_int(z) : 0xFFFFFFFFu;
            if (key_base) {
                const uint32_t kk = valid ? dbits - key_base : 0x1FFFFFFFu;
                reinterpret_cast<uint32_t*>(depth_keys)[pid] = (krange_part ? 0u : ((uint32_t)c << 29)) | kk;
                if (valid) { kmin = min(kmin, kk); kmax = max(kmax, kk); }
            } else
                depth_keys[pid] = ((uint64_t)c << 32) | dbits;
            if (!krange_part) depth_vals[pid] = (int32_t)pid;
        }
        n_vis += valid ? 1 : 0;
    }
    if (krange_part) {
        for (int off = 32; off > 0; off >>= 1) { kmin = min(kmin, (uint32_t)__shfl_down((int)kmin, off)); kmax = max(kmax, (uint32_t)__shfl_down((int)kmax, off)); }
        __shared__ uint32_t redk[8];
        const int w = threadIdx.x >> 6;
        if ((threadIdx.x & 63) == 0) { redk[w] = kmin; redk[4 + w] = kmax; }
        __syncthreads();
        if (threadIdx.x == 0) {
            krange_part[2 * blockIdx.x + 0] = min(min(redk[0], redk[1]), min(redk[2], redk[3]));
            krange_part[2 * blockIdx.x + 1] = max(max(redk[4], redk[5]), max(redk[6], redk[7]));
        }
    }
    if (reg_part) {
        for (int off = 32; off > 0; off >>= 1) { n_vis += __shfl_down(n_vis, off); n_ref += __shfl_down(n_ref, off); }
        __shared__ int redi[8];
        const int w = threadIdx.x >> 6;
        if ((threadIdx.x & 63) == 0) { redi[w] = n_vis; redi[4 + w] = n_ref; }
        __syncthreads();
        if (threadIdx.x == 0) {
            reg_part[4 * blockIdx.x + 2] = (double)((redi[0] + redi[1]) + (redi[2] + redi[3]));
            reg_part[4 * blockIdx.x + 3] = (double)((redi[4] + redi[5]) + (redi[6] + redi[7]));
        }
    }
}

__global__ __launch_bounds__(256) void k_reg_reduce(int n_blocks, const double* __restrict__ reg_part,
                                                    double* __restrict__ reg_sums, int overwrite,
                                                    double* __restrict__ zero_ptr, int zero_n,
                                                    const uint32_t* __restrict__ krange_part,
                                                    uint32_t* __restrict__ krange) {
    for (int i = threadIdx.x; i < zero_n; i += 256) zero_ptr[i] = 0.0;
    if (krange_part) {
        __shared__ uint32_t shk[2][256];
        uint32_t lo = 0xFFFFFFFFu, hi = 0u;
        for (int b = threadIdx.x; b < n_blocks; b += 256) { lo = min(lo, krange_part[2 * b]); hi = max(hi, krange_part[2 * b + 1]); }
        shk[0][threadIdx.x] = lo; shk[1][threadIdx.x] = hi;
        __syncthreads();
        for (int off = 128; off > 0; off >>= 1) {
            if (threadIdx.x < off) {
                shk[0][threadIdx.x] = min(shk[0][threadIdx.x], shk[0][threadIdx.x + off]);
                shk[1][threadIdx.x] = max(shk[1][threadIdx.x], shk[1][threadIdx.x + off]);
            }
            __syncthreads();
        }
        if (threadIdx.x == 0) {
            lo = shk[0][0]; hi = shk[1][0];
            if (hi < lo) { lo = 0u; hi = 0u; }
            const uint32_t top = hi - lo + 1u;
            krange[0] = lo; krange[1] = top;
            krange[2] = top < (1u << 8) ? 1u : top < (1u << 16) ? 2u : top < (1u << 24) ? 3u : 4u;
        }
        __syncthreads();
    }
    __shared__ double sh[4][256];
    double acc[4] = {0, 0, 0, 0};
    for (int b = threadIdx.x; b < n_blocks; b += 256)
        for (int k = 0; k < 4; ++k) acc[k] += reg_part[4 * b + k];
    for (int k = 0; k < 4; ++k) sh[k][threadIdx.x] = acc[k];
    __syncthreads();
    for (int off = 128; off > 0; off >>= 1) {
        if (threadIdx.x < off)
            for (int k = 0; k < 4; ++k) sh[k][threadIdx.x] += sh[k][threadIdx.x + off];
        __syncthreads();
    }
    if (threadIdx.x < 4) reg_sums[threadIdx.x] = (overwrite ? 0.0 : reg_sums[threadIdx.x]) + sh[threadIdx.x][0];
}

int st3r_project_impl(st3r_ctx* ctx, hipStream_t s, int N, int C, const float* means, const float* quats, const float* scales,
                      const float* opacities, const float* sh, int sh_stride, const float* viewmats, const float* Ks,
                      const float* campos, int width, int height, int tile_size, float eps2d, float near_plane,
                      float far_plane, float radius_clip, float* splats, int32_t* tiles_per_gauss, double* reg_sums,
                      uint64_t* depth_keys, int32_t* depth_vals, int tight, uint32_t key_base, void* rects, int rect32,
                      int reg_overwrite, double* zero_ptr, int zero_n, uint32_t* krange) {
    if (N == 0) {
        if (reg_sums && reg_overwrite) HIP_TRY(hipMemsetAsync(reg_sums, 0, sizeof(double) * 4, s));
        if (zero_ptr && zero_n > 0) HIP_TRY(hipMemsetAsync(zero_ptr, 0, sizeof(double) * (size_t)zero_n, s));
        return ST3R_OK;
    }
    int tile_w = (width + tile_size - 1) / tile_size, tile_h = (height + tile_size - 1) / tile_size;
    dim3 grid(ceil_div(N, 256)), block(256);
    size_t shmem = (size_t)C * CAM_STRIDE * sizeof(float);
    double* reg_part = nullptr;
    if (reg_sums) {
        void* p;
        int rc = st3r_arena_get(ctx, SLOT_REG_PART, sizeof(double) * 4 * (size_t)grid.x, &p);
        if (rc) return rc;
        reg_part = (double*)p;
    }
    uint32_t* krange_part = nullptr;
    if (krange && reg_sums) {
        void* p;
        int rc = st3r_arena_get(ctx, SLOT_KRANGE_PART, sizeof(uint32_t) * 2 * (size_t)grid.x, &p);
        if (rc) return rc;
        krange_part = (uint32_t*)p;
    }
    hipLaunchKernelGGL(k_project_sh_fwd, grid, block, shmem, s, N, C, means, quats, scales, opacities, sh, sh_stride,
                       viewmats, Ks, campos, width, height, tile_size, tile_w, tile_h, eps2d, near_plane, far_plane,
                       radius_clip, (float4*)splats, tiles_per_gauss, reg_part, depth_keys, depth_vals, tight, key_base,
                       rects, rect32, krange_part);
    if (reg_sums)
        hipLaunchKernelGGL(k_reg_reduce, dim3(1), dim3(256), 0, s, (int)grid.x, reg_part, reg_sums, reg_overwrite, zero_ptr,
                           zero_ptr ? zero_n : 0, (const uint32_t*)krange_part, krange);
    else if (zero_ptr && zero_n > 0)
        HIP_TRY(hipMemsetAsync(zero_ptr, 0, sizeof(double) * (size_t)zero_n, s));
    LAUNCH_CHECK();
    return ST3R_OK;
}

ST3R_EXPORT int st3r_gs_project_sh(st3r_ctx* ctx, void* stream, int N, int C, const float* means,
                                   const float* quats, const float* scales, const float* opacities,
                                   const float* sh, int sh_stride, const float* viewmats, const float* Ks,
                                   const float* campos, int width, int height, int tile_size, float eps2d,
                                   float near_plane, float far_plane, float radius_clip, float* splats,
                                   int32_t* tiles_per_gauss, double* reg_sums) {
    ARG_CHECK(ctx && N >= 0 && C > 0 && C <= ST3R_MAX_VIEWS && sh_stride >= 12 && width > 0 && height > 0 && tile_size > 0);
    ARG_CHECK(means && quats && scales && opacities && sh && viewmats && Ks && campos && splats && tiles_per_gauss);
    return st3r_project_impl(ctx, (hipStream_t)stream, N, C, means, quats, scales, opacities, sh, sh_stride, viewmats, Ks,
                             campos, width, height, tile_size, eps2d, near_plane, far_plane, radius_clip, splats,
                             tiles_per_gauss, reg_sums, nullptr, nullptr, 0, 0u, nullptr, 0, 0, nullptr, 0, nullptr);
}
```

starst3r_amd/csrc/gs_project_bwd.hip:

```cpp
#include "common.h"
#include "blend_common.h"

#define CAM_STRIDE 32
#ifndef GATHER_WIDE_ABOVE
#define GATHER_WIDE_ABOVE 6
#endif
#define SH_C0 0.2820947917738781f
#define SH_C1 0.48860251190292f

template <bool GATHER>
__global__ __launch_bounds__(256) __attribute__((amdgpu_waves_per_eu(4))) void k_project_sh_bwd(
    int N, int C, const float* __restrict__ means, const float* __restrict__ quats,
    const float* __restrict__ scales, const float* __restrict__ opacities, const float* __restrict__ sh,
    int sh_stride, const float* __restrict__ viewmats, const float* __restrict__ Ks,
    const float* __restrict__ campos, int W, int H, float eps2d, const float4* __restrict__ splats,
    const float4* __restrict__ v_splats, float reg_o_k, float reg_s_k, float* __restrict__ grads, int accumulate,
    int g_begin, int g_end, int range_major, const int32_t* __restrict__ cum, const float* __restrict__ vtile, int stamp,
    unsigned vt_cap, const uint32_t* __restrict__ touch) {
    extern __shared__ float cam[];
    constexpr int ROW = ACC_VALS;
    __shared__ float sVal[GATHER ? 256 * ROW : 1];
    __shared__ float sAcc[GATHER ? 256 * ROW : 1];
    __shared__ int sStart[GATHER ? 4 * 65 : 1];
    for (int c = threadIdx.x; c < C; c += blockDim.x) {
        float* o = cam + c * CAM_STRIDE;
        const float* V = viewmats + 16 * c;
        for (int k = 0; k < 12; ++k) o[k] = V[k];
        const float* K = Ks + 9 * c;
        float fx = K[0], fy = K[4], cx = K[2], cy = K[5];
        o[12] = fx; o[13] = fy; o[14] = cx; o[15] = cy;
        float tan_fovx = 0.5f * (float)W / fx;
        float tan_fovy = 0.5f * (float)H / fy;
        o[16] = ((float)W - cx) / fx + 0.3f * tan_fovx;
        o[17] = cx / fx + 0.3f * tan_fovx;
        o[18] = ((float)H - cy) / fy + 0.3f * tan_fovy;
        o[19] = cy / fy + 0.3f * tan_fovy;
        o[20] = campos[3 * c]; o[21] = campos[3 * c + 1]; o[22] = campos[3 * c + 2];
    }
    __syncthreads();
    const int gbase = g_begin + blockIdx.x * blockDim.x;
    const bool valid = gbase + (int)threadIdx.x < g_end;
    if (!GATHER && !valid) return;
    const int g = valid ? gbase + (int)threadIdx.x : g_end - 1;

    const float mx = means[3 * g], my = means[3 * g + 1], mz = means[3 * g + 2];
    const float opac = opacities[g];
    float qw = quats[4 * g], qx = quats[4 * g + 1], qy = quats[4 * g + 2], qz = quats[4 * g + 3];
    const float s0 = scales[3 * g], s1 = scales[3 * g + 1], s2 = scales[3 * g + 2];
    float k[12];
    const float* kp = sh + (int64_t)g * sh_stride;
#pragma unroll
    for (int i = 0; i < 12; ++i) k[i] = kp[i];
    const float inv_norm = 1.0f / sqrtf(((qw * qw + qx * qx) + qy * qy) + qz * qz);
    qw *= inv_norm; qx *= inv_norm; qy *= inv_norm; qz *= inv_norm;
    const float sc[3] = {s0, s1, s2};
    auto rot_and_m = [&](float (&Rq)[9], float (&M)[9]) {
        float x2 = qx * qx, y2 = qy * qy, z2 = qz * qz, xy = qx * qy, xz = qx * qz, yz = qy * qz;
        float wx = qw * qx, wy = qw * qy, wz = qw * qz;
        Rq[0] = 1.0f - 2.0f * (y2 + z2); Rq[1] = 2.0f * (xy - wz); Rq[2] = 2.0f * (xz + wy);
        Rq[3] = 2.0f * (xy + wz); Rq[4] = 1.0f - 2.0f * (x2 + z2); Rq[5] = 2.0f * (yz - wx);
        Rq[6] = 2.0f * (xz - wy); Rq[7] = 2.0f * (yz + wx); Rq[8] = 1.0f - 2.0f * (x2 + y2);
#pragma unroll
        for (int i = 0; i < 3; ++i)
#pragma unroll
            for (int j = 0; j < 3; ++j) M[i * 3 + j] = Rq[i * 3 + j] * sc[j];
    };
    float cov[6];
    {
        float Rq[9], M[9];
        rot_and_m(Rq, M);
        cov[0] = M[0] * M[0] + M[1] * M[1] + M[2] * M[2];
        cov[1] = M[0] * M[3] + M[1] * M[4] + M[2] * M[5];
        cov[2] = M[0] * M[6] + M[1] * M[7] + M[2] * M[8];
        cov[3] = M[3] * M[3] + M[4] * M[4] + M[5] * M[5];
        cov[4] = M[3] * M[6] + M[4] * M[7] + M[5] * M[8];
        cov[5] = M[6] * M[6] + M[7] * M[7] + M[8] * M[8];
        asm volatile("" : "+v"(cov[0]), "+v"(cov[1]), "+v"(cov[2]), "+v"(cov[3]), "+v"(cov[4]), "+v"(cov[5]));
    }

    float v_mean[3] = {0, 0, 0};
    float vSw[6] = {0, 0, 0, 0, 0, 0};
    float v_k[12];
#pragma unroll
    for (int i = 0; i < 12; ++i) v_k[i] = 0.f;
    float v_opac = 0.f;

    for (int c = 0; c < C; ++c) {
        const int64_t pid = (int64_t)c * N + g;
        float4 g0, g1, g2;
        if (GATHER) {
            const int lane = threadIdx.x & 63, wv = threadIdx.x >> 6;
            float* wval = sVal + wv * (64 * ROW);
            const int my_end = cum[pid];
            const int my_start = !valid ? my_end : (pid == 0 ? 0 : cum[pid - 1]);
            const int s0 = __builtin_amdgcn_readfirstlane(my_start);
            const int s1 = __builtin_amdgcn_readlane(my_end, 63);
            float acc[ACC_VALS];
            float2 q0, q1, q2, q3, q4;
            auto fetch = [&](int u) {
                q0 = q1 = q2 = q3 = q4 = make_float2(0.f, 0.f);
                if (u < s1 && (unsigned)u < vt_cap) {
                    const float2* src = reinterpret_cast<const float2*>(vtile + (int64_t)u * VT_STRIDE);
                    q0 = src[0]; q1 = src[1]; q2 = src[2]; q3 = src[3]; q4 = src[4];
                }
            };
            auto rows_to_lds = [&]() {
                const bool live = __float_as_int(q4.y) == stamp;
                float* row = wval + lane * ROW;
                row[0] = live ? q0.x : 0.f; row[1] = live ? q0.y : 0.f; row[2] = live ? q1.x : 0.f;
                row[3] = live ? q1.y : 0.f; row[4] = live ? q2.x : 0.f; row[5] = live ? q2.y : 0.f;
                row[6] = live ? q3.x : 0.f; row[7] = live ? q3.y : 0.f; row[8] = live ? q4.x : 0.f;
            };
            if (s1 - s0 <= 64 * GATHER_WIDE_ABOVE) {
                if (s1 > s0) fetch(s0 + lane);
#pragma unroll
                for (int k2 = 0; k2 < ACC_VALS; ++k2) acc[k2] = 0.f;
                for (int base = s0; base < s1; base += 64) {
                    rows_to_lds();
                    wave_lds_sync();
                    fetch(base + 64 + lane);
                    const int lo = max(my_start, base) - base, hi = min(my_end, base + 64) - base;
                    for (int r = lo; r < hi; ++r) {
                        const float* src = wval + r * ROW;
#pragma unroll
                        for (int k2 = 0; k2 < ACC_VALS; ++k2) acc[k2] += src[k2];
                    }
                    wave_lds_sync();
                }
            } else {
                float* wacc = sAcc + wv * (64 * ROW);
                int* wst = sStart + wv * 65;
                wst[lane] = my_start;
                if (lane == 63) wst[64] = my_end;
#pragma unroll
                for (int k2 = 0; k2 < ACC_VALS; ++k2) wacc[lane * ROW + k2] = 0.f;
                const uint64_t tmask = touch ? __builtin_amdgcn_ballot_w64(valid && touch[pid] == (uint32_t)stamp) : ~0ull;
                auto meets = [&](int b) {
                    return __builtin_amdgcn_ballot_w64(my_end > my_start && my_start < b + 64 && my_end > b);
                };
                uint64_t pm_next = meets(s0);
                bool have = false;
                if (pm_next & tmask) { fetch(s0 + lane); have = true; }
                for (int base = s0; base < s1; base += 64) {
                    const uint64_t pm = pm_next & tmask;
                    const bool cur = have;
                    if (cur) { rows_to_lds(); wave_lds_sync(); }
                    pm_next = base + 64 < s1 ? meets(base + 64) : 0ull;
                    have = (pm_next & tmask) != 0;
                    if (have) fetch(base + 64 + lane);
                    if (cur) {
                        const int pa = __builtin_ctzll(pm), pb = 63 - __builtin_clzll(pm);
                        const int items = (pb - pa + 1) * ROW;
                        for (int it = lane; it < items; it += 64) {
                            const int q = (it * 7282) >> 16;
                            const int k2 = it - q * ROW, pp = pa + q;
                            const int lo = max(wst[pp], base) - base, hi = min(wst[pp + 1], base + 64) - base;
                            if (hi > lo) {
                                float sum = wacc[pp * ROW + k2];
                                const float* src = wval + k2;
                                int r = lo;
                                for (; r + 4 <= hi; r += 4) {
                                    const float a0 = src[r * ROW], a1 = src[(r + 1) * ROW], a2 = src[(r + 2) * ROW], a3 = src[(r + 3) * ROW];
                                    sum += a0; sum += a1; sum += a2; sum += a3;
                                }
                                for (; r < hi; ++r) sum += src[r * ROW];
                                wacc[pp * ROW + k2] = sum;
                            }
                        }
                        wave_lds_sync();
                    }
                }
                wave_lds_sync();
#pragma unroll
                for (int k2 = 0; k2 < ACC_VALS; ++k2) acc[k2] = wacc[lane * ROW + k2];
                wave_lds_sync();
            }
            g0 = make_float4(acc[0], acc[1], acc[2], acc[3]);
            g1 = make_float4(acc[4], acc[5], acc[6], acc[7]);
            g2 = make_float4(acc[8], 0.f, 0.f, 0.f);
            if (!valid) continue;
        }
        const float4 r2 = splats[pid * 3 + 2];
        if (__float_as_int(r2.z) <= 0) continue;
        const float4 r0 = splats[pid * 3 + 0];
        const float4 r1 = splats[pid * 3 + 1];
        if (!GATHER) {
            g0 = v_splats[pid * 3 + 0];
            g1 = v_splats[pid * 3 + 1];
            g2 = v_splats[pid * 3 + 2];
        }
        const float* o = cam + c * CAM_STRIDE;
        const float R[9] = {o[0], o[1], o[2], o[4], o[5], o[6], o[8], o[9], o[10]};
        v_opac += g0.z;
        {
            float dx = mx - o[20], dy = my - o[21], dz = mz - o[22];
            float nrm = sqrtf(dx * dx + dy * dy + dz * dz);
            float inrm = 1.0f / nrm;
            float ux = dx * inrm, uy = dy * inrm, uz = dz * inrm;
            const float vcol[3] = {g1.z, g1.w, g2.x};
            const float colf[3] = {r1.z, r1.w, r2.x};
            float vdx = 0.f, vdy = 0.f, vdz = 0.f;
#pragma unroll
            for (int ch = 0; ch < 3; ++ch) {
                float pre = SH_C0 * k[ch] + SH_C1 * ((-uy * k[3 + ch] + uz * k[6 + ch]) - ux * k[9 + ch]) + 0.5f;
                float vc = (colf[ch] > 0.0f || pre >= 0.0f) ? vcol[ch] : 0.0f;
                v_k[ch] += SH_C0 * vc;
                v_k[3 + ch] += -SH_C1 * uy * vc;
                v_k[6 + ch] += SH_C1 * uz * vc;
                v_k[9 + ch] += -SH_C1 * ux * vc;
                vdx += -SH_C1 * k[9 + ch] * vc;
                vdy += -SH_C1 * k[3 + ch] * vc;
                vdz += SH_C1 * k[6 + ch] * vc;
            }
            float dotp = vdx * ux + vdy * uy + vdz * uz;
            v_mean[0] += (vdx - dotp * ux) * inrm;
            v_mean[1] += (vdy - dotp * uy) * inrm;
            v_mean[2] += (vdz - dotp * uz) * inrm;
        }
        const float x = R[0] * mx + R[1] * my + R[2] * mz + o[3];
        const float y = R[3] * mx + R[4] * my + R[5] * mz + o[7];
        const float z = R[6] * mx + R[7] * my + R[8] * mz + o[11];
        float T[9];
#pragma unroll
        for (int i = 0; i < 3; ++i) {
            T[i * 3 + 0] = R[i * 3] * cov[0] + R[i * 3 + 1] * cov[1] + R[i * 3 + 2] * cov[2];
            T[i * 3 + 1] = R[i * 3] * cov[1] + R[i * 3 + 1] * cov[3] + R[i * 3 + 2] * cov[4];
            T[i * 3 + 2] = R[i * 3] * cov[2] + R[i * 3 + 1] * cov[4] + R[i * 3 + 2] * cov[5];
        }
        const float S00 = T[0] * R[0] + T[1] * R[1] + T[2] * R[2];
        const float S01 = T[0] * R[3] + T[1] * R[4] + T[2] * R[5];
        const float S02 = T[0] * R[6] + T[1] * R[7] + T[2] * R[8];
        const float S11 = T[3] * R[3] + T[4] * R[4] + T[5] * R[5];
        const float S12 = T[3] * R[6] + T[4] * R[7] + T[5] * R[8];
        const float S22 = T[6] * R[6] + T[7] * R[7] + T[8] * R[8];
        const float fx = o[12], fy = o[13];
        const float rz = 1.0f / z, rz2 = rz * rz, rz3 = rz2 * rz;
        const float xr = x * rz, yr = y * rz;
        const bool x_in = (xr <= o[16]) && (xr >= -o[17]);
        const bool y_in = (yr <= o[18]) && (yr >= -o[19]);
        const float tx = z * fminf(o[16], fmaxf(-o[17], xr));
        const float ty = z * fminf(o[18], fmaxf(-o[19], yr));
        const float a = fx * rz, cj = -fx * tx * rz2, b = fy * rz, d = -fy * ty * rz2;
        const float A = r0.w, B = r1.x, Cc = r1.y;
        const float vA = g0.w, vB = 0.5f * g1.x, vC = g1.y;
        const float X00 = A * vA + B * vB, X01 = A * vB + B * vC;
        const float X10 = B * vA + Cc * vB, X11 = B * vB + Cc * vC;
        const float G00 = -(X00 * A + X01 * B);
        const float G01 = -0.5f * ((X00 * B + X01 * Cc) + (X10 * A + X11 * B));
        const float G11 = -(X10 * B + X11 * Cc);
        const float GJ00 = G00 * a, GJ01 = G01 * b, GJ02 = G00 * cj + G01 * d;
        const float GJ10 = G01 * a, GJ11 = G11 * b, GJ12 = G01 * cj + G11 * d;
        const float vS00 = a * GJ00, vS01 = a * GJ01, vS02 = a * GJ02;
        const float vS11 = b * GJ11, vS12 = b * GJ12, vS22 = cj * GJ02 + d * GJ12;
        const float vJ00 = 2.0f * (GJ00 * S00 + GJ01 * S01 + GJ02 * S02);
        const float vJ02 = 2.0f * (GJ00 * S02 + GJ01 * S12 + GJ02 * S22);
        const float vJ11 = 2.0f * (GJ10 * S01 + GJ11 * S11 + GJ12 * S12);
        const float vJ12 = 2.0f * (GJ10 * S02 + GJ11 * S12 + GJ12 * S22);
        const float vm2x = g0.x, vm2y = g0.y;
        float vpx = fx * rz * vm2x;
        float vpy = fy * rz * vm2y;
        float vpz = -(fx * x * vm2x + fy * y * vm2y) * rz2;
        vpz += -fx * rz2 * vJ00 - fy * rz2 * vJ11;
        if (x_in) { vpx += -fx * rz2 * vJ02; vpz += 2.0f * fx * x * rz3 * vJ02; }
        else { vpz += fx * tx * rz3 * vJ02; }
        if (y_in) { vpy += -fy * rz2 * vJ12; vpz += 2.0f * fy * y * rz3 * vJ12; }
        else { vpz += fy * ty * rz3 * vJ12; }
        v_mean[0] += R[0] * vpx + R[3] * vpy + R[6] * vpz;
        v_mean[1] += R[1] * vpx + R[4] * vpy + R[7] * vpz;
        v_mean[2] += R[2] * vpx + R[5] * vpy + R[8] * vpz;
        float U[9];
        const float vSm[9] = {vS00, vS01, vS02, vS01, vS11, vS12, vS02, vS12, vS22};
#pragma unroll
        for (int i = 0; i < 3; ++i)
#pragma unroll
            for (int j = 0; j < 3; ++j)
                U[i * 3 + j] = vSm[i * 3] * R[j] + vSm[i * 3 + 1] * R[3 + j] + vSm[i * 3 + 2] * R[6 + j];
        vSw[0] += R[0] * U[0] + R[3] * U[3] + R[6] * U[6];
        vSw[1] += R[0] * U[1] + R[3] * U[4] + R[6] * U[7];
        vSw[2] += R[0] * U[2] + R[3] * U[5] + R[6] * U[8];
        vSw[3] += R[1] * U[1] + R[4] * U[4] + R[7] * U[7];
        vSw[4] += R[1] * U[2] + R[4] * U[5] + R[7] * U[8];
        vSw[5] += R[2] * U[2] + R[5] * U[5] + R[8] * U[8];
    }

    if (GATHER && !valid) return;
    float Rq[9], M[9];
    asm volatile("" : "+v"(qw), "+v"(qx), "+v"(qy), "+v"(qz));
    rot_and_m(Rq, M);
    const float W9[9] = {vSw[0], vSw[1], vSw[2], vSw[1], vSw[3], vSw[4], vSw[2], vSw[4], vSw[5]};
    float vM[9];
#pragma unroll
    for (int r = 0; r < 3; ++r)
#pragma unroll
        for (int s = 0; s < 3; ++s)
            vM[r * 3 + s] = 2.0f * (W9[r * 3] * M[s] + W9[r * 3 + 1] * M[3 + s] + W9[r * 3 + 2] * M[6 + s]);
    float v_scale[3], vR[9];
#pragma unroll
    for (int s = 0; s < 3; ++s) {
        v_scale[s] = Rq[s] * vM[s] + Rq[3 + s] * vM[3 + s] + Rq[6 + s] * vM[6 + s];
        vR[s] = vM[s] * sc[s]; vR[3 + s] = vM[3 + s] * sc[s]; vR[6 + s] = vM[6 + s] * sc[s];
    }
    float vq0 = 2.0f * (qx * (vR[7] - vR[5]) + qy * (vR[2] - vR[6]) + qz * (vR[3] - vR[1]));
    float vq1 = 2.0f * (-2.0f * qx * (vR[4] + vR[8]) + qy * (vR[3] + vR[1]) + qz * (vR[6] + vR[2]) + qw * (vR[7] - vR[5]));
    float vq2 = 2.0f * (qx * (vR[3] + vR[1]) - 2.0f * qy * (vR[0] + vR[8]) + qz * (vR[7] + vR[5]) + qw * (vR[2] - vR[6]));
    float vq3 = 2.0f * (qx * (vR[6] + vR[2]) + qy * (vR[7] + vR[5]) - 2.0f * qz * (vR[0] + vR[4]) + qw * (vR[3] - vR[1]));
    const float dq = vq0 * qw + vq1 * qx + vq2 * qy + vq3 * qz;
    vq0 = (vq0 - dq * qw) * inv_norm; vq1 = (vq1 - dq * qx) * inv_norm;
    vq2 = (vq2 - dq * qy) * inv_norm; vq3 = (vq3 - dq * qz) * inv_norm;

    const float sg = 1.0f / (1.0f + __expf(-opac));
    v_opac += reg_o_k * sg * (1.0f - sg);
    v_scale[0] += reg_s_k * __expf(s0);
    v_scale[1] += reg_s_k * __expf(s1);
    v_scale[2] += reg_s_k * __expf(s2);

    const int64_t Nl = range_major ? g_end - g_begin : N;
    float* gb = range_major ? grads + (int64_t)23 * g_begin : grads;
    const int gw = range_major ? g - g_begin : g;
    float* gm = gb; float* gq = gb + 3 * Nl; float* gs = gb + 7 * Nl;
    float* go = gb + 10 * Nl; float* gsh = gb + 11 * Nl;
    if (accumulate) {
        v_mean[0] += gm[3 * gw]; v_mean[1] += gm[3 * gw + 1]; v_mean[2] += gm[3 * gw + 2];
        vq0 += gq[4 * gw]; vq1 += gq[4 * gw + 1]; vq2 += gq[4 * gw + 2]; vq3 += gq[4 * gw + 3];
        v_scale[0] += gs[3 * gw]; v_scale[1] += gs[3 * gw + 1]; v_scale[2] += gs[3 * gw + 2];
        v_opac += go[gw];
#pragma unroll
        for (int i = 0; i < 12; ++i) v_k[i] += gsh[(int64_t)gw * 12 + i];
    }
    gm[3 * gw] = v_mean[0]; gm[3 * gw + 1] = v_mean[1]; gm[3 * gw + 2] = v_mean[2];
    gq[4 * gw] = vq0; gq[4 * gw + 1] = vq1; gq[4 * gw + 2] = vq2; gq[4 * gw + 3] = vq3;
    gs[3 * gw] = v_scale[0]; gs[3 * gw + 1] = v_scale[1]; gs[3 * gw + 2] = v_scale[2];
    go[gw] = v_opac;
#pragma unroll
    for (int i = 0; i < 12; ++i) gsh[(int64_t)gw * 12 + i] = v_k[i];
}

int st3r_project_sh_bwd_impl(hipStream_t s, int N, int C, const float* means, const float* quats, const float* scales,
                             const float* opacities, const float* sh, int sh_stride, const float* viewmats,
                             const float* Ks, const float* campos, int width, int height, float eps2d,
                             const float* splats, const float* v_splats, float reg_views, float opac_fac,
                             float scale_fac, float* grads, bool accumulate, int g_begin, int g_end, bool range_major,
                             const st3r_vtile_ref* slots) {
    if (g_end < 0) g_end = N;
    if (N == 0 || g_end <= g_begin) return ST3R_OK;
    float reg_o_k = reg_views * opac_fac / (float)N;
    float reg_s_k = reg_views * scale_fac / (3.0f * (float)N);
    size_t shmem = (size_t)C * CAM_STRIDE * sizeof(float);
    if (slots)
        hipLaunchKernelGGL(k_project_sh_bwd<true>, dim3(ceil_div(g_end - g_begin, 256)), dim3(256), shmem, s, N, C, means,
                           quats, scales, opacities, sh, sh_stride, viewmats, Ks, campos, width, height, eps2d,
                           (const float4*)splats, (const float4*)nullptr, reg_o_k, reg_s_k, grads, accumulate ? 1 : 0, g_begin,
                           g_end, range_major ? 1 : 0, slots->cum, slots->vtile, slots->stamp, slots->vt_cap, slots->touch);
    else
        hipLaunchKernelGGL(k_project_sh_bwd<false>, dim3(ceil_div(g_end - g_begin, 256)), dim3(256), shmem, s, N, C, means,
                           quats, scales, opacities, sh, sh_stride, viewmats, Ks, campos, width, height, eps2d,
                           (const float4*)splats, (const float4*)v_splats, reg_o_k, reg_s_k, grads, accumulate ? 1 : 0, g_begin,
                           g_end, range_major ? 1 : 0, (const int32_t*)nullptr, (const float*)nullptr, 0, 0u, (const uint32_t*)nullptr);
    LAUNCH_CHECK();
    return ST3R_OK;
}

ST3R_EXPORT int st3r_gs_project_sh_bwd(st3r_ctx* ctx, void* stream, int N, int C, const float* means,
                                       const float* quats, const float* scales, const float* opacities,
                                       const float* sh, int sh_stride, const float* viewmats, const float* Ks,
                                       const float* campos, int width, int height, float eps2d,
                                       const float* splats, const float* v_splats, float reg_views,
                                       float opac_fac, float scale_fac, float* grads) {
    ARG_CHECK(ctx && N >= 0 && C > 0 && C <= ST3R_MAX_VIEWS && sh_stride >= 12);
    ARG_CHECK(means && quats && scales && opacities && sh && viewmats && Ks && campos && splats && v_splats && grads);
    return st3r_project_sh_bwd_impl((hipStream_t)stream, N, C, means, quats, scales, opacities, sh, sh_stride, viewmats,
                                    Ks, campos, width, height, eps2d, splats, v_splats, reg_views, opac_fac, scale_fac,
                                    grads, false, 0, -1, false, nullptr);
}
```

Measured before the change: 191.2.

## Fuse intersection-count prefix scan into projection kernel via decoupled lookback

Runs the per-pair tile-count prefix scan inside the forward projection kernel, one decoupled-lookback chain per camera, and writes cum, rectbase and per-camera base offsets directly. This removes the separate scan kernel launch and its extra pass over per-pair data. Because cum is now per-camera relative, blend backward and the projection backward gather add a cam_base offset. In exchange the projection kernel uses more LDS and spin-waits on lookback, which can lower occupancy, and the path only applies to 8 or fewer views.

```diff
diff --git a/starst3r_amd/csrc/api.hip b/starst3r_amd/csrc/api.hip
--- a/starst3r_amd/csrc/api.hip
+++ b/starst3r_amd/csrc/api.hip
@@ -89,10 +89,10 @@
 }
 
 ST3R_EXPORT int st3r_ctx_peek(st3r_ctx* ctx, void* stream, int which, void* dst, int64_t bytes) {
-    ARG_CHECK(ctx && dst && bytes >= 0 && which >= 0 && which <= 10);
-    static const int slots[11] = {SLOT_VALS_B, SLOT_OFFSETS, SLOT_SPLATS, SLOT_CUM,
+    ARG_CHECK(ctx && dst && bytes >= 0 && which >= 0 && which <= 12);
+    static const int slots[13] = {SLOT_VALS_B, SLOT_OFFSETS, SLOT_SPLATS, SLOT_CUM,
                                   SLOT_MCMC_CUM, SLOT_MCMC_DEAD, SLOT_MCMC_SAMPLED, SLOT_MCMC_COUNT,
-                                  SLOT_RGB, SLOT_ALPHA, SLOT_COUNTS};
+                                  SLOT_RGB, SLOT_ALPHA, SLOT_COUNTS, SLOT_RECTBASE, SLOT_CAM_BASE};
     ARG_CHECK((size_t)bytes <= ctx->slot_bytes[slots[which]]);
     HIP_TRY(hipMemcpyAsync(dst, ctx->slot_ptr[slots[which]], (size_t)bytes, hipMemcpyDeviceToDevice,
                            (hipStream_t)stream));
@@ -178,7 +178,7 @@
                       const float* campos, int width, int height, int tile_size, float eps2d, float near_plane,
                       float far_plane, float radius_clip, float* splats, int32_t* tiles_per_gauss, double* reg_sums,
                       uint64_t* depth_keys, int32_t* depth_vals, int tight, uint32_t key_base, void* rects, int rect32,
-                      int reg_overwrite, double* zero_ptr, int zero_n, uint32_t* krange);
+                      int reg_overwrite, double* zero_ptr, int zero_n, uint32_t* krange, st3r_proj_scan* fuse);
 int st3r_sort_depth_seg_impl(st3r_ctx* ctx, hipStream_t s, int64_t N, int C, uint32_t* keys_in, int32_t* vals_in,
                              uint32_t* keys_out, int32_t* vals_out, const uint32_t* krange);
 int st3r_isect_emit_chain_impl(st3r_ctx* ctx, hipStream_t s, int N, int C, const int32_t* perm, const void* rects,
@@ -202,7 +202,7 @@
                         const float* alpha, const int32_t* last_ids, const float* v_rgb, const float* v_alpha,
                         const int32_t* cum, const uint64_t* rects, const uint64_t* rectbase, int tight, int64_t n_pairs,
                         float* v_splats,
-                        bool end_in_offsets, st3r_vtile_ref* defer);
+                        bool end_in_offsets, st3r_vtile_ref* defer, const int32_t* cam_base);
 int st3r_project_sh_bwd_impl(hipStream_t s, int N, int C, const float* means, const float* quats, const float* scales,
                              const float* opacities, const float* sh, int sh_stride, const float* viewmats,
                              const float* Ks, const float* campos, int width, int height, float eps2d,
@@ -279,6 +279,7 @@
 
 struct RasterOut {
     float* splats; int32_t* offsets; int32_t* flat; int32_t* cum; const uint64_t* rects; uint64_t* rectbase;
+    const int32_t* cam_base;
     int64_t n_isects, n_records, n_isects_ref, n_visible; int tile_w, tile_h;
 };
 
@@ -311,6 +312,16 @@
     int32_t* counts = nullptr;
     { int rc_ = st3r_counts_buffer(ctx, s, &counts); if (rc_) return rc_; }
     uint32_t* const krange = (key32 && reg_sums && !records_in && !(ctx->debug_flags & 4)) ? (uint32_t*)(counts + 8) : nullptr;
+    uint64_t* rectbase = nullptr;
+    if (tile_w <= 1023 && tile_h <= 1023 && !(ctx->debug_flags & 64)) {
+        GET(SLOT_RECTBASE, uint64_t, n_pairs, rb);
+        rectbase = rb;
+    }
+    const int64_t sig = ((int64_t)N << 34) ^ ((int64_t)C << 26) ^ ((int64_t)W << 13) ^ (int64_t)H;
+    const bool async = allow_async && ctx->isect_hint > 0 && ctx->hint_sig == sig;
+    st3r_proj_scan fuse_{cum, rectbase, async ? counts : nullptr, async ? (int32_t*)(ctx->pinned + 8) : nullptr, nullptr, nullptr};
+    st3r_proj_scan* const fuse =
+        (!records_in && rectbase && C <= ST3R_PROJ_SCAN_MAX_VIEWS && !(ctx->debug_flags & (2 | 4096))) ? &fuse_ : nullptr;
     st3r_prof_begin(ctx, s, STG_PROJECT);
     const uint32_t key_base = key32 ? near_bits : 0u;
     int rc = records_in
@@ -318,7 +329,7 @@
                                              key_base, rects, rect32)
                  : st3r_project_impl(ctx, s, N, C, means, quats, scales, opacities, sh, sh_stride, viewmats, Ks, campos,
                                      W, H, tile, 0.3f, near_plane, far_plane, 0.0f, splats, nullptr, reg_sums, dkeys_a,
-                                     dvals_a, tight, key_base, rects, rect32, 1, loss_sums, 2 * C, krange);
+                                     dvals_a, tight, key_base, rects, rect32, 1, loss_sums, 2 * C, krange, fuse);
     if (!rc && records_in && loss_sums) HIP_TRY(hipMemsetAsync(loss_sums, 0, sizeof(double) * 2 * (size_t)C, s));
     st3r_prof_end(ctx, s, STG_PROJECT);
     if (rc) return rc;
@@ -332,17 +343,11 @@
     if (rc) return rc;
     int64_t n_isects = 0;
     st3r_prof_begin(ctx, s, STG_SCAN);
-    uint64_t* rectbase = nullptr;
-    if (tile_w <= 1023 && tile_h <= 1023 && !(ctx->debug_flags & 64)) {
-        GET(SLOT_RECTBASE, uint64_t, n_pairs, rb);
-        rectbase = rb;
-    }
     const int32_t* n_dev = nullptr;
-    const int64_t sig = ((int64_t)N << 34) ^ ((int64_t)C << 26) ^ ((int64_t)W << 13) ^ (int64_t)H;
-    const bool async = allow_async && ctx->isect_hint > 0 && ctx->hint_sig == sig;
-    int32_t* total_dev = nullptr;
-    rc = st3r_isect_scan_impl(ctx, s, n_pairs, nullptr, cum, nullptr, rects, rect32, rectbase, &total_dev,
-                              async ? counts : nullptr, async ? (int32_t*)(ctx->pinned + 8) : nullptr);
+    int32_t* total_dev = fuse ? fuse->total_dev : nullptr;
+    if (!fuse)
+        rc = st3r_isect_scan_impl(ctx, s, n_pairs, nullptr, cum, nullptr, rects, rect32, rectbase, &total_dev,
+                                  async ? counts : nullptr, async ? (int32_t*)(ctx->pinned + 8) : nullptr);
     st3r_prof_end(ctx, s, STG_SCAN);
     if (rc) return rc;
     if (async) {
@@ -388,7 +393,7 @@
     st3r_prof_end(ctx, s, STG_OFFSETS);
     if (rc) return rc;
     o->splats = splats; o->offsets = offsets; o->flat = vals_b; o->cum = cum; o->rects = rect32 ? nullptr : rects;
-    o->rectbase = rectbase;
+    o->rectbase = rectbase; o->cam_base = fuse ? fuse->cam_base : nullptr;
     o->n_isects = n_isects;
     o->tile_w = tile_w; o->tile_h = tile_h;
     return ST3R_OK;
@@ -435,7 +440,7 @@
     rc = st3r_blend_bwd_impl(ctx, s, C, W, H, ro.tile_w, ro.tile_h, ro.splats, ro.offsets, ro.flat, ro.n_isects, alpha,
                              last, v_rgb, nullptr, ro.cum, (ctx->debug_flags & 2) ? nullptr : ro.rects,
                              (ctx->debug_flags & 2) ? nullptr : ro.rectbase, 1, n_pairs, v_splats,
-                             eio, slots);
+                             eio, slots, ro.cam_base);
     st3r_prof_end(ctx, s, STG_BLEND_BWD);
     if (rc) return rc;
     st3r_prof_begin(ctx, s, STG_PROJECT_BWD);
@@ -556,7 +561,7 @@
     if (rc) return rc;
     st3r_prof_begin(ctx, s, STG_BLEND_BWD);
     rc = st3r_blend_bwd_impl(ctx, s, C, W, H, ro.tile_w, ro.tile_h, ro.splats, ro.offsets, ro.flat, ro.n_isects, alpha,
-                             last, v_rgb, nullptr, ro.cum, ro.rects, ro.rectbase, 1, n_pairs, v_records, true, nullptr);
+                             last, v_rgb, nullptr, ro.cum, ro.rects, ro.rectbase, 1, n_pairs, v_records, true, nullptr, nullptr);
     st3r_prof_end(ctx, s, STG_BLEND_BWD);
     if (rc) return rc;
     const int Hi = H - 10, Wi = W - 10;
diff --git a/starst3r_amd/csrc/chain_scan.h b/starst3r_amd/csrc/chain_scan.h
--- /dev/null
+++ b/starst3r_amd/csrc/chain_scan.h
@@ -0,0 +1,65 @@
+#pragma once
+#include "common.h"
+
+__device__ __forceinline__ int wave_incl_scan(int v) {
+    const int lane = threadIdx.x & 63;
+#pragma unroll
+    for (int off = 1; off < 64; off <<= 1) {
+        int t = __shfl_up(v, off);
+        if (lane >= off) v += t;
+    }
+    return v;
+}
+
+__device__ __forceinline__ int block_incl_scan(int v, int* total) {
+    __shared__ int wsum[4];
+    const int lane = threadIdx.x & 63, w = threadIdx.x >> 6;
+    int inc = wave_incl_scan(v);
+    if (lane == 63) wsum[w] = inc;
+    __syncthreads();
+    int base = 0;
+#pragma unroll
+    for (int i = 0; i < 4; ++i) base += (i < w) ? wsum[i] : 0;
+    *total = wsum[0] + wsum[1] + wsum[2] + wsum[3];
+    __syncthreads();
+    return inc + base;
+}
+
+typedef unsigned long long u64;
+#define SC_VALUE_MASK 0xFFFFFFFFFFFFull
+__device__ __forceinline__ u64 sc_word(u64 flag, uint32_t gen, u64 v) { return (flag << 62) | ((u64)gen << 48) | (v & SC_VALUE_MASK); }
+
+__device__ __forceinline__ u64 chain_lookback256(const u64* st, int k, uint32_t gen, u64* s_part, int* s_near) {
+    const int t = threadIdx.x, lane = t & 63, w = t >> 6;
+    u64 excl = 0;
+    for (int t0 = k - 1;; t0 -= 256) {
+        const int tt = t0 - t;
+        u64 wd = sc_word(2, gen, 0);
+        if (tt >= 0) {
+            unsigned spins = 0;
+            for (;;) {
+                wd = __hip_atomic_load(st + tt, __ATOMIC_RELAXED, __HIP_MEMORY_SCOPE_AGENT);
+                if ((wd >> 62) != 0 && (uint32_t)((wd >> 48) & 0x3FFF) == gen) break;
+                __builtin_amdgcn_s_sleep(1);
+                if (++spins > (1u << 26)) __builtin_trap();
+            }
+        }
+        const u64 incm = __ballot((wd >> 62) == 2);
+        const int nearest = incm ? __builtin_ctzll(incm) : 64;
+        u64 val = lane <= nearest ? (wd & SC_VALUE_MASK) : 0ull;
+#pragma unroll
+        for (int off = 32; off > 0; off >>= 1) val += __shfl_down(val, off);
+        if (lane == 0) { s_part[w] = val; s_near[w] = nearest; }
+        __syncthreads();
+        bool done = false;
+#pragma unroll
+        for (int ww = 0; ww < 4; ++ww)
+            if (!done) { excl += s_part[ww]; done = s_near[ww] < 64; }
+        __syncthreads();
+        if (done) break;
+    }
+    return excl;
+}
+
+struct ChainCtl { uint32_t* tickets; int32_t* total; u64* status; uint32_t gen; };
+int st3r_chain_ctl(st3r_ctx* ctx, hipStream_t s, int64_t nwords, ChainCtl* c);
diff --git a/starst3r_amd/csrc/common.h b/starst3r_amd/csrc/common.h
--- a/starst3r_amd/csrc/common.h
+++ b/starst3r_amd/csrc/common.h
@@ -76,6 +76,7 @@
     SLOT_POSE_PART,
     SLOT_VTILE_DEPTH,
     SLOT_DEPTH_PART,
+    SLOT_CAM_BASE,
     SLOT_COUNT
 };
 
@@ -98,7 +99,13 @@
 
 #define ST3R_SPLIT_VIEWS 1000
 
-struct st3r_vtile_ref { const int32_t* cum; const float* vtile; int stamp; unsigned vt_cap; const uint32_t* touch; };
+struct st3r_vtile_ref { const int32_t* cum; const float* vtile; int stamp; unsigned vt_cap; const uint32_t* touch; const int32_t* cam_base; };
+
+#define ST3R_PROJ_SCAN_MAX_VIEWS 8
+struct st3r_proj_scan {
+    int32_t* cum; uint64_t* rectbase; int32_t* total_copy; int32_t* total_host;
+    const int32_t* cam_base; int32_t* total_dev;
+};
 
 struct st3r_ctx {
     int device;
diff --git a/starst3r_amd/csrc/gs_blend.hip b/starst3r_amd/csrc/gs_blend.hip
--- a/starst3r_amd/csrc/gs_blend.hip
+++ b/starst3r_amd/csrc/gs_blend.hip
@@ -261,6 +261,11 @@
     const TileGeom g = tile_geom(C, W, H, tile_w, tile_h, offsets, n_isects);
     const int nb = tile_nb[g.lb];
     if (nb == 0) return;
+    if (rectbase && (tight & 2)) {
+        const unsigned b = (unsigned)cum[g.cam];
+        vtile += (int64_t)b * VT_STRIDE;
+        vt_cap = b < vt_cap ? vt_cap - b : 0u;
+    }
     const int w = threadIdx.x >> 6, lane = threadIdx.x & 63;
     const int64_t p = ((int64_t)g.cam * H + g.i) * W + g.j;
     float T_final = 1.0f, vr = 0.f, vg = 0.f, vb = 0.f, va = 0.f;
@@ -334,7 +339,7 @@
                     x0 = (int)(r & 0xFFFF); y0 = (int)((r >> 16) & 0xFFFF); rw = (int)((r >> 32) & 0xFFFF);
                 } else {
                     TileRect tr = ref_tile_rect(a.x, a.y, (float)__float_as_int(c.z), 16, tile_w, tile_h);
-                    if (tight) tr = tight_tile_rect(tr, a.x, a.y, a.z, a.w, b.x, b.y);
+                    if (tight & 1) tr = tight_tile_rect(tr, a.x, a.y, a.z, a.w, b.x, b.y);
                     x0 = tr.x0; y0 = tr.y0; rw = tr.x1 - tr.x0;
                 }
                 const int cum_excl = my_id == 0 ? 0 : cum[my_id - 1];
@@ -473,8 +478,9 @@
                         const float* splats, const int32_t* offsets, const int32_t* flat, int64_t n_isects,
                         const float* alpha, const int32_t* last_ids, const float* v_rgb, const float* v_alpha,
                         const int32_t* cum, const uint64_t* rects, const uint64_t* rectbase, int tight, int64_t n_pairs,
-                        float* v_splats, bool end_in_offsets, st3r_vtile_ref* defer) {
-    if (defer) *defer = st3r_vtile_ref{cum, nullptr, 0, 0u, nullptr};
+                        float* v_splats, bool end_in_offsets, st3r_vtile_ref* defer, const int32_t* cam_base) {
+    if (cam_base && !(rectbase && defer)) { st3r_set_error("blend backward: per-camera slot bases need rectbase and a deferred gather"); return ST3R_ERR_INVALID; }
+    if (defer) *defer = st3r_vtile_ref{cum, nullptr, 0, 0u, nullptr, cam_base};
     if (n_isects == 0) {
         if (!defer) HIP_TRY(hipMemsetAsync(v_splats, 0, sizeof(float) * ST3R_SPLAT_STRIDE * (size_t)n_pairs, s));
         return ST3R_OK;
@@ -505,21 +511,23 @@
     const int stamp = ++ctx->bwd_stamp;
     const int total = C * tile_w * tile_h;
     const unsigned vt_cap = (unsigned)(ctx->slot_bytes[SLOT_VTILE] / (sizeof(float) * VT_STRIDE));
+    const int32_t* const kcum = cam_base ? cam_base : cum;
+    tight = (tight ? 1 : 0) | (cam_base ? 2 : 0);
     if (v_alpha)
         hipLaunchKernelGGL(k_blend_bwd<true>, dim3(total), dim3(BLK), 0, s, C, W, H, tile_w, tile_h,
                            (const float4*)splats, offsets, flat, end_in_offsets ? -1 : (int)n_isects, alpha, last_ids, v_rgb,
-                           v_alpha, cmask, words, tile_nb, cum, rects, rectbase, tight, vtile, stamp, vt_cap);
+                           v_alpha, cmask, words, tile_nb, kcum, rects, rectbase, tight, vtile, stamp, vt_cap);
     else if (touch)
         hipLaunchKernelGGL((k_blend_bwd<false, true>), dim3(total), dim3(BLK), 0, s, C, W, H, tile_w, tile_h,
                            (const float4*)splats, offsets, flat, end_in_offsets ? -1 : (int)n_isects, alpha, last_ids, v_rgb,
-                           v_alpha, cmask, words, tile_nb, cum, reinterpret_cast<const uint64_t*>(touch), rectbase, tight, vtile,
+                           v_alpha, cmask, words, tile_nb, kcum, reinterpret_cast<const uint64_t*>(touch), rectbase, tight, vtile,
                            stamp, vt_cap);
     else
         hipLaunchKernelGGL(k_blend_bwd<false>, dim3(total), dim3(BLK), 0, s, C, W, H, tile_w, tile_h,
                            (const float4*)splats, offsets, flat, end_in_offsets ? -1 : (int)n_isects, alpha, last_ids, v_rgb,
-                           v_alpha, cmask, words, tile_nb, cum, rects, rectbase, tight, vtile, stamp, vt_cap);
+                           v_alpha, cmask, words, tile_nb, kcum, rects, rectbase, tight, vtile, stamp, vt_cap);
     LAUNCH_CHECK();
-    if (defer) { *defer = st3r_vtile_ref{cum, vtile, stamp, vt_cap, touch}; return ST3R_OK; }
+    if (defer) { *defer = st3r_vtile_ref{cum, vtile, stamp, vt_cap, touch, cam_base}; return ST3R_OK; }
     hipLaunchKernelGGL(k_gather_vtile, dim3(ceil_div(n_pairs, 256)), dim3(256), 0, s, n_pairs, cum, vtile, stamp, vt_cap,
                        (float4*)v_splats);
     LAUNCH_CHECK();
@@ -537,5 +545,5 @@
     ARG_CHECK(n_isects >= 0 && n_isects < 2147483647LL && (n_isects == 0 || flatten_ids));
     return st3r_blend_bwd_impl(ctx, (hipStream_t)stream, C, width, height, tile_w, tile_h, splats, offsets,
                                flatten_ids, n_isects, alpha, last_ids, v_rgb, v_alpha, cum_tiles, nullptr, nullptr, 0, n_pairs,
-                               v_splats, false, nullptr);
-}
+                               v_splats, false, nullptr, nullptr);
+}
diff --git a/starst3r_amd/csrc/gs_isect.hip b/starst3r_amd/csrc/gs_isect.hip
--- a/starst3r_amd/csrc/gs_isect.hip
+++ b/starst3r_amd/csrc/gs_isect.hip
@@ -1,71 +1,12 @@
 #include "common.h"
 #include "tile_rect.h"
+#include "chain_scan.h"
 
 #define SCAN_THREADS 256
 #define SCAN_ITEMS 16
 #define SCAN_TILE (SCAN_THREADS * SCAN_ITEMS)
 
-__device__ __forceinline__ int wave_incl_scan(int v) {
-    const int lane = threadIdx.x & 63;
-#pragma unroll
-    for (int off = 1; off < 64; off <<= 1) {
-        int t = __shfl_up(v, off);
-        if (lane >= off) v += t;
-    }
-    return v;
-}
-
-__device__ __forceinline__ int block_incl_scan(int v, int* total) {
-    __shared__ int wsum[4];
-    const int lane = threadIdx.x & 63, w = threadIdx.x >> 6;
-    int inc = wave_incl_scan(v);
-    if (lane == 63) wsum[w] = inc;
-    __syncthreads();
-    int base = 0;
-#pragma unroll
-    for (int i = 0; i < 4; ++i) base += (i < w) ? wsum[i] : 0;
-    *total = wsum[0] + wsum[1] + wsum[2] + wsum[3];
-    __syncthreads();
-    return inc + base;
-}
-
-typedef unsigned long long u64;
 #define SCAN_PAD(i) ((i) + ((i) >> 5))
-#define SC_VALUE_MASK 0xFFFFFFFFFFFFull
-__device__ __forceinline__ u64 sc_word(u64 flag, uint32_t gen, u64 v) { return (flag << 62) | ((u64)gen << 48) | (v & SC_VALUE_MASK); }
-
-__device__ __forceinline__ u64 chain_lookback256(const u64* st, int k, uint32_t gen, u64* s_part, int* s_near) {
-    const int t = threadIdx.x, lane = t & 63, w = t >> 6;
-    u64 excl = 0;
-    for (int t0 = k - 1;; t0 -= 256) {
-        const int tt = t0 - t;
-        u64 wd = sc_word(2, gen, 0);
-        if (tt >= 0) {
-            unsigned spins = 0;
-            for (;;) {
-                wd = __hip_atomic_load(st + tt, __ATOMIC_RELAXED, __HIP_MEMORY_SCOPE_AGENT);
-                if ((wd >> 62) != 0 && (uint32_t)((wd >> 48) & 0x3FFF) == gen) break;
-                __builtin_amdgcn_s_sleep(1);
-                if (++spins > (1u << 26)) __builtin_trap();
-            }
-        }
-        const u64 incm = __ballot((wd >> 62) == 2);
-        const int nearest = incm ? __builtin_ctzll(incm) : 64;
-        u64 val = lane <= nearest ? (wd & SC_VALUE_MASK) : 0ull;
-#pragma unroll
-        for (int off = 32; off > 0; off >>= 1) val += __shfl_down(val, off);
-        if (lane == 0) { s_part[w] = val; s_near[w] = nearest; }
-        __syncthreads();
-        bool done = false;
-#pragma unroll
-        for (int ww = 0; ww < 4; ++ww)
-            if (!done) { excl += s_part[ww]; done = s_near[ww] < 64; }
-        __syncthreads();
-        if (done) break;
-    }
-    return excl;
-}
-
 template <bool RECTS, bool PACK>
 __global__ __launch_bounds__(SCAN_THREADS) void k_scan_chained(const int32_t* in, const void* __restrict__ rects,
                                                                int rect32, int64_t n, int32_t* out,
@@ -148,8 +89,7 @@
     }
 }
 
-struct ChainCtl { uint32_t* tickets; int32_t* total; u64* status; uint32_t gen; };
-static int chain_ctl(st3r_ctx* ctx, hipStream_t s, int64_t nwords, ChainCtl* c) {
+int st3r_chain_ctl(st3r_ctx* ctx, hipStream_t s, int64_t nwords, ChainCtl* c) {
     void* p; int grown = 0;
     int rc = st3r_arena_get2(ctx, SLOT_SCAN_CHAIN, sizeof(u64) * ((size_t)nwords + 16), &p, &grown);
     if (rc) return rc;
@@ -170,7 +110,7 @@
                             int32_t* total_host = nullptr) {
     const int ntiles = ceil_div(n, SCAN_TILE);
     ChainCtl c;
-    int rc = chain_ctl(ctx, s, ntiles, &c);
+    int rc = st3r_chain_ctl(ctx, s, ntiles, &c);
     if (rc) return rc;
 #define SCAN_LAUNCH(R, P)                                                                                                \
     hipLaunchKernelGGL((k_scan_chained<R, P>), dim3(ntiles), dim3(SCAN_THREADS), 0, s, in, rects, rect32, n, out, pack_out, \
diff --git a/starst3r_amd/csrc/gs_project.hip b/starst3r_amd/csrc/gs_project.hip
--- a/starst3r_amd/csrc/gs_project.hip
+++ b/starst3r_amd/csrc/gs_project.hip
@@ -1,5 +1,6 @@
 #include "common.h"
 #include "tile_rect.h"
+#include "chain_scan.h"
 
 #define CAM_STRIDE 32
 
@@ -10,7 +11,15 @@
 #define SH_C0 0.2820947917738781f
 #define SH_C1 0.48860251190292f
 
-__global__ __launch_bounds__(256) void k_project_sh_fwd(
+struct ProjScan {
+    u64* status; uint32_t* ticket; uint32_t gen; int n_blocks;
+    int32_t* cum; uint64_t* rectbase;
+    int32_t* cam_base;
+    int32_t* total_copy; int32_t* total_host;
+};
+
+template <bool FUSED>
+__global__ __launch_bounds__(256) __attribute__((amdgpu_waves_per_eu(7))) void k_project_sh_fwd(
     int N, int C, const float* __restrict__ means, const float* __restrict__ quats,
     const float* __restrict__ scales, const float* __restrict__ opacities, const float* __restrict__ sh,
     int sh_stride, const float* __restrict__ viewmats, const float* __restrict__ Ks,
@@ -18,9 +27,17 @@
     float near_plane, float far_plane, float radius_clip, float4* __restrict__ splats,
     int32_t* __restrict__ tiles_per_gauss, double* __restrict__ reg_part,
     uint64_t* __restrict__ depth_keys, int32_t* __restrict__ depth_vals, int tight, uint32_t key_base,
-    void* __restrict__ rects, int rect32, uint32_t* __restrict__ krange_part) {
+    void* __restrict__ rects, int rect32, uint32_t* __restrict__ krange_part, ProjScan sc) {
     extern __shared__ float cam[];
     __shared__ float red[8];
+    __shared__ uint32_t s_blk;
+    __shared__ u64 s_part[4];
+    __shared__ int s_near[4];
+    __shared__ u64 s_before;
+    if (FUSED && threadIdx.x == 0) {
+        s_blk = atomicAdd(sc.ticket + (sc.gen & 1u), 1u);
+        if (s_blk == 0) __hip_atomic_store(sc.ticket + ((sc.gen & 1u) ^ 1u), 0u, __ATOMIC_RELAXED, __HIP_MEMORY_SCOPE_AGENT);
+    }
     for (int c = threadIdx.x; c < C; c += blockDim.x) {
         float* o = cam + c * CAM_STRIDE;
         const float* V = viewmats + 16 * c;
@@ -38,7 +55,8 @@
     }
     __syncthreads();
 
-    const int g = blockIdx.x * blockDim.x + threadIdx.x;
+    const int blk = FUSED ? (int)s_blk : (int)blockIdx.x;
+    const int g = blk * blockDim.x + threadIdx.x;
     const bool active = g < N;
     float mx = 0, my = 0, mz = 0, opac = 0;
     float cov0 = 0, cov1 = 0, cov2 = 0, cov3 = 0, cov4 = 0, cov5 = 0;
@@ -81,12 +99,16 @@
         if ((threadIdx.x & 63) == 0) { red[w] = reg_o; red[4 + w] = reg_s; }
         __syncthreads();
         if (threadIdx.x == 0) {
-            reg_part[4 * blockIdx.x + 0] = (double)((red[0] + red[1]) + (red[2] + red[3]));
-            reg_part[4 * blockIdx.x + 1] = (double)((red[4] + red[5]) + (red[6] + red[7]));
+            reg_part[4 * blk + 0] = (double)((red[0] + red[1]) + (red[2] + red[3]));
+            reg_part[4 * blk + 1] = (double)((red[4] + red[5]) + (red[6] + red[7]));
         }
     }
     int n_vis = 0, n_ref = 0;
     uint32_t kmin = 0xFFFFFFFFu, kmax = 0u;
+    if (FUSED && threadIdx.x == 0) s_before = 0;
+    u64* pairw = reinterpret_cast<u64*>(cam + C * CAM_STRIDE);
+    if (FUSED && !active)
+        for (int c = 0; c < C; ++c) pairw[c * 256 + threadIdx.x] = 0;
     for (int c = 0; active && c < C; ++c) {
         const float* o = cam + c * CAM_STRIDE;
         const float R00 = o[0], R01 = o[1], R02 = o[2], t0 = o[3];
@@ -183,6 +205,43 @@
             if (!krange_part) depth_vals[pid] = (int32_t)pid;
         }
         n_vis += valid ? 1 : 0;
+        if (FUSED)
+            pairw[c * 256 + threadIdx.x] =
+                ntiles == 0 ? 0ull : ((u64)(uint32_t)ntiles << 32) | (uint32_t)(tr.x0 & 0x3FF) | ((uint32_t)(tr.y0 & 0x3FF) << 10) |
+                                         ((uint32_t)((tr.x1 - tr.x0) & 0x3FF) << 20);
+    }
+    for (int c = 0; FUSED && c < C; ++c) {
+        const u64 pw = pairw[c * 256 + threadIdx.x];
+        const int ntiles = (int)(pw >> 32);
+        const uint32_t geo = (uint32_t)pw;
+        const int64_t pid = (int64_t)c * N + g;
+        int tot;
+        const int inc = block_incl_scan(ntiles, &tot);
+        u64* st = sc.status + (size_t)c * sc.n_blocks;
+        u64 excl = 0;
+        if (blk == 0) {
+            if (threadIdx.x == 0) __hip_atomic_store(st, sc_word(2, sc.gen, (u64)(uint32_t)tot), __ATOMIC_RELAXED, __HIP_MEMORY_SCOPE_AGENT);
+        } else {
+            if (threadIdx.x == 0) __hip_atomic_store(st + blk, sc_word(1, sc.gen, (u64)(uint32_t)tot), __ATOMIC_RELAXED, __HIP_MEMORY_SCOPE_AGENT);
+            excl = chain_lookback256(st, blk, sc.gen, s_part, s_near);
+            if (threadIdx.x == 0)
+                __hip_atomic_store(st + blk, sc_word(2, sc.gen, excl + (u64)(uint32_t)tot), __ATOMIC_RELAXED, __HIP_MEMORY_SCOPE_AGENT);
+        }
+        if (blk == sc.n_blocks - 1 && threadIdx.x == 0) {
+            sc.cam_base[c] = (int32_t)(uint32_t)s_before;
+            s_before += excl + (u64)(uint32_t)tot;
+        }
+        if (active) {
+            const uint32_t end = (uint32_t)excl + (uint32_t)inc;
+            sc.cum[pid] = (int32_t)end;
+            sc.rectbase[pid] = ((uint64_t)(end - (uint32_t)ntiles) << 32) | geo;
+        }
+    }
+    if (FUSED && blk == sc.n_blocks - 1 && threadIdx.x == 0) {
+        const int32_t total = s_before > 2147483647ull ? -1 : (int32_t)s_before;
+        sc.cam_base[C] = total;
+        if (sc.total_copy) sc.total_copy[0] = total;
+        if (sc.total_host) __hip_atomic_store(sc.total_host, total, __ATOMIC_RELAXED, __HIP_MEMORY_SCOPE_SYSTEM);
     }
     if (krange_part) {
         for (int off = 32; off > 0; off >>= 1) { kmin = min(kmin, (uint32_t)__shfl_down((int)kmin, off)); kmax = max(kmax, (uint32_t)__shfl_down((int)kmax, off)); }
@@ -191,8 +250,8 @@
         if ((threadIdx.x & 63) == 0) { redk[w] = kmin; redk[4 + w] = kmax; }
         __syncthreads();
         if (threadIdx.x == 0) {
-            krange_part[2 * blockIdx.x + 0] = min(min(redk[0], redk[1]), min(redk[2], redk[3]));
-            krange_part[2 * blockIdx.x + 1] = max(max(redk[4], redk[5]), max(redk[6], redk[7]));
+            krange_part[2 * blk + 0] = min(min(redk[0], redk[1]), min(redk[2], redk[3]));
+            krange_part[2 * blk + 1] = max(max(redk[4], redk[5]), max(redk[6], redk[7]));
         }
     }
     if (reg_part) {
@@ -202,8 +261,8 @@
         if ((threadIdx.x & 63) == 0) { redi[w] = n_vis; redi[4 + w] = n_ref; }
         __syncthreads();
         if (threadIdx.x == 0) {
-            reg_part[4 * blockIdx.x + 2] = (double)((redi[0] + redi[1]) + (redi[2] + redi[3]));
-            reg_part[4 * blockIdx.x + 3] = (double)((redi[4] + redi[5]) + (redi[6] + redi[7]));
+            reg_part[4 * blk + 2] = (double)((redi[0] + redi[1]) + (redi[2] + redi[3]));
+            reg_part[4 * blk + 3] = (double)((redi[4] + redi[5]) + (redi[6] + redi[7]));
         }
     }
 }
@@ -255,7 +314,7 @@
                       const float* campos, int width, int height, int tile_size, float eps2d, float near_plane,
                       float far_plane, float radius_clip, float* splats, int32_t* tiles_per_gauss, double* reg_sums,
                       uint64_t* depth_keys, int32_t* depth_vals, int tight, uint32_t key_base, void* rects, int rect32,
-                      int reg_overwrite, double* zero_ptr, int zero_n, uint32_t* krange) {
+                      int reg_overwrite, double* zero_ptr, int zero_n, uint32_t* krange, st3r_proj_scan* fuse) {
     if (N == 0) {
         if (reg_sums && reg_overwrite) HIP_TRY(hipMemsetAsync(reg_sums, 0, sizeof(double) * 4, s));
         if (zero_ptr && zero_n > 0) HIP_TRY(hipMemsetAsync(zero_ptr, 0, sizeof(double) * (size_t)zero_n, s));
@@ -264,6 +323,7 @@
     int tile_w = (width + tile_size - 1) / tile_size, tile_h = (height + tile_size - 1) / tile_size;
     dim3 grid(ceil_div(N, 256)), block(256);
     size_t shmem = (size_t)C * CAM_STRIDE * sizeof(float);
+    if (fuse) shmem += (size_t)C * 256 * sizeof(u64);
     double* reg_part = nullptr;
     if (reg_sums) {
         void* p;
@@ -278,10 +338,26 @@
         if (rc) return rc;
         krange_part = (uint32_t*)p;
     }
-    hipLaunchKernelGGL(k_project_sh_fwd, grid, block, shmem, s, N, C, means, quats, scales, opacities, sh, sh_stride,
-                       viewmats, Ks, campos, width, height, tile_size, tile_w, tile_h, eps2d, near_plane, far_plane,
-                       radius_clip, (float4*)splats, tiles_per_gauss, reg_part, depth_keys, depth_vals, tight, key_base,
-                       rects, rect32, krange_part);
+    ProjScan sc{};
+    if (fuse) {
+        ChainCtl c;
+        int rc = st3r_chain_ctl(ctx, s, (int64_t)C * grid.x, &c);
+        if (rc) return rc;
+        void* p;
+        rc = st3r_arena_get(ctx, SLOT_CAM_BASE, sizeof(int32_t) * ((size_t)C + 1), &p);
+        if (rc) return rc;
+        sc = ProjScan{c.status, c.tickets, c.gen, (int)grid.x, fuse->cum, fuse->rectbase, (int32_t*)p,
+                      fuse->total_copy, fuse->total_host};
+        fuse->cam_base = (const int32_t*)p; fuse->total_dev = (int32_t*)p + C;
+    }
+#define PROJECT_LAUNCH(F)                                                                                                 \
+    hipLaunchKernelGGL(k_project_sh_fwd<F>, grid, block, shmem, s, N, C, means, quats, scales, opacities, sh, sh_stride,  \
+                       viewmats, Ks, campos, width, height, tile_size, tile_w, tile_h, eps2d, near_plane, far_plane,      \
+                       radius_clip, (float4*)splats, tiles_per_gauss, reg_part, depth_keys, depth_vals, tight, key_base,  \
+                       rects, rect32, krange_part, sc)
+    if (fuse) PROJECT_LAUNCH(true);
+    else PROJECT_LAUNCH(false);
+#undef PROJECT_LAUNCH
     if (reg_sums)
         hipLaunchKernelGGL(k_reg_reduce, dim3(1), dim3(256), 0, s, (int)grid.x, reg_part, reg_sums, reg_overwrite, zero_ptr,
                            zero_ptr ? zero_n : 0, (const uint32_t*)krange_part, krange);
@@ -301,5 +377,5 @@
     ARG_CHECK(means && quats && scales && opacities && sh && viewmats && Ks && campos && splats && tiles_per_gauss);
     return st3r_project_impl(ctx, (hipStream_t)stream, N, C, means, quats, scales, opacities, sh, sh_stride, viewmats, Ks,
                              campos, width, height, tile_size, eps2d, near_plane, far_plane, radius_clip, splats,
-                             tiles_per_gauss, reg_sums, nullptr, nullptr, 0, 0u, nullptr, 0, 0, nullptr, 0, nullptr);
-}
+                             tiles_per_gauss, reg_sums, nullptr, nullptr, 0, 0u, nullptr, 0, 0, nullptr, 0, nullptr, nullptr);
+}
diff --git a/starst3r_amd/csrc/gs_project_bwd.hip b/starst3r_amd/csrc/gs_project_bwd.hip
--- a/starst3r_amd/csrc/gs_project_bwd.hip
+++ b/starst3r_amd/csrc/gs_project_bwd.hip
@@ -16,7 +16,7 @@
     const float* __restrict__ campos, int W, int H, float eps2d, const float4* __restrict__ splats,
     const float4* __restrict__ v_splats, float reg_o_k, float reg_s_k, float* __restrict__ grads, int accumulate,
     int g_begin, int g_end, int range_major, const int32_t* __restrict__ cum, const float* __restrict__ vtile, int stamp,
-    unsigned vt_cap, const uint32_t* __restrict__ touch) {
+    unsigned vt_cap, const uint32_t* __restrict__ touch, const int32_t* __restrict__ cam_base) {
     extern __shared__ float cam[];
     constexpr int ROW = ACC_VALS;
     __shared__ float sVal[GATHER ? 256 * ROW : 1];
@@ -91,8 +91,9 @@
         if (GATHER) {
             const int lane = threadIdx.x & 63, wv = threadIdx.x >> 6;
             float* wval = sVal + wv * (64 * ROW);
-            const int my_end = cum[pid];
-            const int my_start = !valid ? my_end : (pid == 0 ? 0 : cum[pid - 1]);
+            const int cb = cam_base ? cam_base[c] : 0;
+            const int my_end = cum[pid] + cb;
+            const int my_start = !valid ? my_end : ((cam_base ? g == 0 : pid == 0) ? cb : cum[pid - 1] + cb);
             const int s0 = __builtin_amdgcn_readfirstlane(my_start);
             const int s1 = __builtin_amdgcn_readlane(my_end, 63);
             float acc[ACC_VALS];
@@ -350,12 +351,14 @@
         hipLaunchKernelGGL(k_project_sh_bwd<true>, dim3(ceil_div(g_end - g_begin, 256)), dim3(256), shmem, s, N, C, means,
                            quats, scales, opacities, sh, sh_stride, viewmats, Ks, campos, width, height, eps2d,
                            (const float4*)splats, (const float4*)nullptr, reg_o_k, reg_s_k, grads, accumulate ? 1 : 0, g_begin,
-                           g_end, range_major ? 1 : 0, slots->cum, slots->vtile, slots->stamp, slots->vt_cap, slots->touch);
+                           g_end, range_major ? 1 : 0, slots->cum, slots->vtile, slots->stamp, slots->vt_cap, slots->touch,
+                           slots->cam_base);
     else
         hipLaunchKernelGGL(k_project_sh_bwd<false>, dim3(ceil_div(g_end - g_begin, 256)), dim3(256), shmem, s, N, C, means,
                            quats, scales, opacities, sh, sh_stride, viewmats, Ks, campos, width, height, eps2d,
                            (const float4*)splats, (const float4*)v_splats, reg_o_k, reg_s_k, grads, accumulate ? 1 : 0, g_begin,
-                           g_end, range_major ? 1 : 0, (const int32_t*)nullptr, (const float*)nullptr, 0, 0u, (const uint32_t*)nullptr);
+                           g_end, range_major ? 1 : 0, (const int32_t*)nullptr, (const float*)nullptr, 0, 0u, (const uint32_t*)nullptr,
+                           (const int32_t*)nullptr);
     LAUNCH_CHECK();
     return ST3R_OK;
 }
```

New measurement: 182.1. -4.8%, worse.
